# NVlabs/intrinsic3d

Measured on AMD Instinct MI355X. Metric: Gauss-Newton iterations/s at the finest SDF level, higher is better.
Workload: dtype f32

## Files before the change

intrinsic3d_amd/csrc/device/build.hip:

```cpp
#include <type_traits>
#include "kernels.hpp"
#include "reduce_device.hpp"

namespace i3d {

typedef float v4f_row __attribute__((ext_vector_type(4)));
typedef float v2f_row __attribute__((ext_vector_type(2)));
typedef float f2 __attribute__((ext_vector_type(2)));
static __device__ inline void st_row2(float2* p, float a, float b) { v2f_row v; v.x = a; v.y = b; __builtin_nontemporal_store(v, reinterpret_cast<v2f_row*>(p)); }
static __device__ inline void st_row(float4* p, float a, float b, float c, float d) { v4f_row v; v.x = a; v.y = b; v.z = c; v.w = d; __builtin_nontemporal_store(v, reinterpret_cast<v4f_row*>(p)); }

typedef float f4u __attribute__((ext_vector_type(4), aligned(4)));
typedef const __attribute__((address_space(1))) f4u* gf4u_ptr;
typedef const __attribute__((address_space(1))) float* gf_ptr;

constexpr int Q_LDS_STRIDE = 296;
struct PointShared {
    double P[3];
    double B;
    float n[3];
    float inv_len;
    float s;
    float Ls;
    float dLs[3];
// ... 449 lines not shown
                    const f2 e0 = c * (au * dxk0 + av * (y0 * r2 + c2 * dxk0)), e1 = c * (au * dxk1 + av * (y0 * r4 + c2 * dxk1)), e2 = c * (au * dxk2 + av * (y0 * r6 + c2 * dxk2));
                    const f2 e3 = c * (au * dxk3 + av * (c2 * dxk3 + (r2 + 2.0f * y0 * y0))), e4 = c * (au * dxk4 + av * (2.0f * xd * y0 + c2 * dxk4));
                    J[P_DIST + 0] -= e0.x + e0.y; J[P_DIST + 1] -= e1.x + e1.y; J[P_DIST + 2] -= e2.x + e2.y; J[P_DIST + 3] -= e3.x + e3.y; J[P_DIST + 4] -= e4.x + e4.y;
                }
                J[P_POSE + 0] = -(Wx * jr[0] + Wy * jr[3] + Wz * jr[6]);
                J[P_POSE + 1] = -(Wx * jr[1] + Wy * jr[4] + Wz * jr[7]);
                J[P_POSE + 2] = -(Wx * jr[2] + Wy * jr[5] + Wz * jr[8]);
                float finz = 0.0f;
#pragma unroll
                for (int i = 0; i < P_TOTAL; ++i) finz = __builtin_fmaf(J[i], 0.0f, finz);
                if (!(finz == 0.0f)) continue;
#pragma unroll
                for (int gq = 0; gq < 7; ++gq)
                    st_row(&r.rows[row_index(a, nout, gq, r.slots)], J[4 * gq], J[4 * gq + 1], J[4 * gq + 2], J[4 * gq + 3]);
                const size_t ro = row_scalar_index(a, nout, r.slots);
                st_row2(&r.row_jt()[row_jt_index(a, nout, r.slots)], J[28], __int_as_float(f | (vox_free ? ROW_FREE_BIT : 0)));
                st_row2(&r.row_wr[ro], roww, (float)res);
                ++nout;
            }
            }
        }
        if (WITH_J) {
            r.nrows[a] = (uint8_t)nout;
        }
        }
    }
#ifdef I3D_COST_MULTI_PROBE
    if (!WITH_J && probe_extra) cost = 0.0;
#endif
    if (!WITH_J) block_partial_d(cost, cost_out, 1, 0);
}

void launch_build(hipStream_t st, GridView g, RowView r, OptParams p, const FrameConst* frames, bool with_jacobian, double* cost_out, double* scratch,
                  const double* cam9, const LmState* lm) {
    if (r.nC <= 0) { if (!with_jacobian && cost_out) (void)hipMemsetAsync(cost_out, 0, sizeof(double), st); return; }
#ifdef I3D_COST_MULTI_PROBE
    const int blocks = with_jacobian ? (r.nC + 255) / 256 : (((r.nC + 255) / 256 + 7) / 8) * 8 * I3D_COST_MULTI_PROBE;
#else
    const int blocks = (r.nC + 255) / 256;
#endif
    double* const cost_dst = cost_out; cost_out = scratch;
    const size_t lds = (size_t)p.K * sizeof(FrameHot), qlds = (size_t)256 * Q_LDS_STRIDE;
    if (with_jacobian) {
#ifdef I3D_BUILD_VALUE_PROBE
        if (BUILD_PROBE_WAVES > 2) {
            if (!set_dynamic_lds((const void*)k_build<true, true, 2>, "k_build<true> value probe", lds, p.K)) return;
            k_build<true, true, 2><<<blocks, 256, lds, st>>>(g, r, p, frames, cost_out, nullptr, nullptr);
            return;
        }
#endif
        if (!set_dynamic_lds((const void*)k_build<true, false, 2>, "k_build<true>", qlds, p.K)) return;
        k_build<true, false, 2><<<blocks, 256, qlds, st>>>(g, r, p, frames, cost_out, nullptr, nullptr);
    } else {
        if (lds <= 48 * 1024) k_build<false, true, 2><<<blocks, 256, lds, st>>>(g, r, p, frames, cost_out, cam9, lm);
        else k_build<false, false, 2><<<blocks, 256, 0, st>>>(g, r, p, frames, cost_out, cam9, lm);
    }
    if (!with_jacobian) launch_reduce_partials(st, scratch, blocks, 1, cost_dst, nullptr, true);
}

template <bool COST>
__global__ void __launch_bounds__(256) k_weight_sums(RowView r, GridView g, double* partials) {
    double s0 = 0, s1 = 0, s2 = 0, s3 = 0, n0 = 0, n3 = 0, na = 0, c0 = 0, c1 = 0, c2 = 0, c3 = 0;
    const int N = g.N;
    for (int a = r.own0 + blockIdx.x * blockDim.x + threadIdx.x; a < r.own1 && a < r.A; a += gridDim.x * blockDim.x) {
        if (!(r.aflags[a] & F_ACTIVE)) continue;
        na += 1.0;
        const int nr = r.nrows[a];
        for (int k = 0; k < nr; ++k) {
            const float2 wr = r.row_wr[row_scalar_index(a, k, r.slots)]; const float w = wr.x;
            s0 += (double)w; if (w != 0.0f) n0 += 1.0;
            if (COST && (__float_as_int(r.row_jt()[row_jt_index(a, k, r.slots)].y) & ROW_FREE_BIT)) c0 += (double)w * ((double)wr.y * (double)wr.y);
        }
        const uint8_t rf = r.regflags[a];
        if (rf & 1) s1 += 1.0;
        if (rf & 2) s2 += 1.0;
        const int s = COST ? r.alist[a] : 0;
        const uint8_t eafree = COST ? r.ea_free[a] : 0;
        const bool er = COST && (rf & 1) && (rf & 8), es = COST && (rf & 2) && (rf & 16);
        int ring[6];
        if (er || eafree) {
#pragma unroll
            for (int d = 0; d < 6; ++d) ring[d] = g.nbr[(size_t)d * N + s];
        }
        if (er || es) {
            const double xs = g.x_sdf[s];
            if (er) {
                const double dxx = g.x_sdf[ring[0]] + g.x_sdf[ring[1]] - 2.0 * xs, dyy = g.x_sdf[ring[2]] + g.x_sdf[ring[3]] - 2.0 * xs, dzz = g.x_sdf[ring[4]] + g.x_sdf[ring[5]] - 2.0 * xs;
                const double lap = dxx + dyy + dzz; c1 += lap * lap;
            }
            if (es) { double e = xs - g.sdf0[s]; if (e == 0.0) e = 0.0000001; c2 += e * e; }
// ... 24 lines not shown
```

intrinsic3d_amd/csrc/device/gradcol.hip:

```cpp
#include "kernels.hpp"
#include "reduce_device.hpp"
#include "wave_ops.hpp"

namespace i3d {

constexpr int GC_THREADS = 384, GC_NW = GC_THREADS / 64, GC_TC = 16, GC_NPV = 27, GC_NCAM = 34;
constexpr int GC_D_CAMW = 4, GC_D_TAG = GC_D_CAMW + ((GC_NW * (GC_NCAM + 0) + 3) & ~3), GC_D_VAL = GC_D_TAG + GC_NW * GC_TC, GC_D0 = GC_D_VAL + GC_NW * GC_TC * GC_NPV;

__device__ constexpr int8_t GC_TRI_I[21] = {0, 0, 0, 0, 0, 0, 1, 1, 1, 1, 1, 2, 2, 2, 2, 3, 3, 3, 4, 4, 5};
__device__ constexpr int8_t GC_TRI_J[21] = {0, 1, 2, 3, 4, 5, 1, 2, 3, 4, 5, 2, 3, 4, 5, 3, 4, 5, 4, 5, 5};

#ifndef GC_OCC
#define GC_OCC 2
#endif
__global__ void __launch_bounds__(GC_THREADS, GC_OCC) k_eg_gradcol(GridView g, RowView r, OptParams p, GradColBuffers b, int tiles_per_block) {
    extern __shared__ float lds[];
    const int K = p.K; const size_t Acap = r.Acap;
    const int rs = (GC_NPV * K) | 1;
    const int nacc = GC_D0 + rs + GC_NCAM;
    for (int i = threadIdx.x; i < nacc; i += GC_THREADS) lds[i] = (i >= GC_D_TAG && i < GC_D_VAL) ? __int_as_float(-1) : 0.0f;
    __syncthreads();
    const int wave = __builtin_amdgcn_readfirstlane((int)(threadIdx.x >> 6));
    const int o_tag = GC_D_TAG + wave * GC_TC, o_val = GC_D_VAL + wave * (GC_TC * GC_NPV);
    int tcount = 0;
// ... 121 lines not shown
#pragma unroll
    for (int i = 0; i < GC_NCAM; ++i) {
        float v = i < 9 ? cam9[i] : camb[i - 9];
        for (int o = 32; o > 0; o >>= 1) v += __shfl_down(v, o, 64);
        if ((threadIdx.x & 63) == 0) lds[GC_D_CAMW + wave * GC_NCAM + i] = v;
    }
    __syncthreads();
    if (threadIdx.x < GC_NCAM) { float v = 0.0f; for (int w = 0; w < GC_NW; ++w) v += lds[GC_D_CAMW + w * GC_NCAM + threadIdx.x]; cam_acc[threadIdx.x] = v; }
    __syncthreads();
    float* const rowg = b.part + (size_t)blockIdx.x * b.part_stride;
    float* const rowc = rowg + b.col_off;
    for (int i = threadIdx.x; i < 6 * K; i += GC_THREADS) { const int f = i / 6; rowg[i] = lds[GC_D0 + GC_NPV * f + (i - 6 * f)]; }
    for (int i = threadIdx.x; i < 21 * K; i += GC_THREADS) { const int f = i / 21; rowc[i] = lds[GC_D0 + GC_NPV * f + 6 + (i - 21 * f)]; }
    if (threadIdx.x < 9) rowg[6 * K + threadIdx.x] = cam_acc[threadIdx.x];
    if (threadIdx.x < 34) {
        const int i = threadIdx.x;
        constexpr int8_t DIAG[9] = {0, 4, 7, 9, 10, 15, 19, 22, 24};
        rowc[21 * K + i] = i < 9 ? cam_acc[9 + DIAG[i]] : cam_acc[i];
    }
}

int launch_eg_gradcol(hipStream_t st, GridView g, RowView r, OptParams p, GradColBuffers b) {
    if (r.nC <= 0) return 0;
    static int num_cu = 0;
    if (!num_cu) { int dev = 0; (void)hipGetDevice(&dev); hipDeviceProp_t pr; (void)hipGetDeviceProperties(&pr, dev); num_cu = pr.multiProcessorCount > 0 ? pr.multiProcessorCount : 256; }
    const int ntiles = (r.nC + GC_THREADS - 1) / GC_THREADS;
    const int want = 2 * num_cu;
    const int blocks = ntiles < want ? ntiles : want;
    const int tiles_per_block = (ntiles + blocks - 1) / blocks;
    const size_t n = (size_t)(GC_D0 + ((GC_NPV * p.K) | 1) + GC_NCAM) * sizeof(float);
    if (!set_dynamic_lds((const void*)k_eg_gradcol, "k_eg_gradcol", n, p.K)) return 0;
    const int used = (ntiles + tiles_per_block - 1) / tiles_per_block;
    k_eg_gradcol<<<used, GC_THREADS, n, st>>>(g, r, p, b, tiles_per_block);
    launch_reduce_partials(st, b.cost_partials, used, 1, b.cost_out, nullptr);
    return used;
}

}
```

intrinsic3d_amd/csrc/device/kernels.hpp:

```cpp
#pragma once
#include "common.hpp"
#include "p2p_device.hpp"

namespace i3d {

struct HashTable { unsigned long long* keys; int* vals; unsigned int mask; };
void launch_sort_keys(hipStream_t st, int N, const int* keys_xyz , unsigned long long* sort_keys, int* iota);
void launch_permute_grid(hipStream_t st, int N, const int* perm, const int* keys_xyz, const double* sdf, const double* sdf_ref,
                         const double* alb, const float* w, const uint8_t* rgb,
                         int* cx, int* cy, int* cz, int* rank, double* sdf0, double* x_sdf, double* x_alb, float* f_sdf, float* f_alb,
                         float* weight, uchar4* color);
void launch_hash_build(hipStream_t st, int N, const int* cx, const int* cy, const int* cz, HashTable t);
void launch_nbr_build(hipStream_t st, int N, const int* cx, const int* cy, const int* cz, HashTable t, int* nbr);
void launch_classify(hipStream_t st, GridView g, OptParams p, int* active_flag);
void launch_compact(hipStream_t st, int N, const int* active_flag, const int* active_scan, const uint8_t* flags, int* aidx, int* alist, uint8_t* aflags);
void launch_partition_blocks(hipStream_t st, GridView g, int A, int* alist, uint8_t* aflags, int* aidx);
void launch_group_rows(hipStream_t st, int A, const uint8_t* nrows, int* gmax);
void launch_anbr(hipStream_t st, int N, int A, int Acap, const int* alist, const int* nbr, const int* aidx, int* anbr);
void launch_scatter_sh(hipStream_t st, int N, const int* rank, const double* sh_visit , float* sh );
void launch_gather_visit(hipStream_t st, int N, const int* rank, const double* x_sdf, const double* x_alb, double* out_sdf, double* out_alb);
void launch_update_fields(hipStream_t st, int N, const int* rank, const double* sdf_ref, const double* alb, const uint8_t* rgb,
                          double* x_sdf, double* x_alb, float* f_sdf, float* f_alb, uchar4* color);

void launch_observe(hipStream_t st, GridView g, RowView r, OptParams p, const FrameConst* frames, const unsigned* cull_mask = nullptr, bool prefilter = false);
constexpr int CULL_BLOCK = 8, CULL_MAX_LEVELS = 12;
struct CullPyramid { int levels, cells; int bw[CULL_MAX_LEVELS], bh[CULL_MAX_LEVELS], off[CULL_MAX_LEVELS]; };
CullPyramid cull_pyramid(int w, int h);
void launch_depth_blocks(hipStream_t st, const FrameConst* frames, int K, int w, int h, float2* out);
void launch_group_cull(hipStream_t st, GridView g, RowView r, OptParams p, const FrameConst* frames, const float2* dblocks, float4* bounds, unsigned* mask);

void launch_build(hipStream_t st, GridView g, RowView r, OptParams p, const FrameConst* frames, bool with_jacobian, double* cost_out , double* scratch,
                  const double* cam9 = nullptr, const LmState* lm = nullptr);
void launch_weight_sums(hipStream_t st, RowView r, GridView g, bool with_cost, double* sums13 , double* scratch);

enum PassMode { PASS_GRAD = 0, PASS_JTJP = 1, PASS_COLNORM = 2 };
struct Seg2 { size_t off0, off1; int n; };
struct PassBuffers {
    float* C;
    float* treg;
    double* shared;
    double* blocks;
    float* part; int part_stride;
};
struct GradColBuffers {
    float* Cg; float* Cc;
    float* tregg; float* tregc;
    float* part; int part_stride;
    int col_off;
    double* cost_partials; double* cost_out;
};
int  launch_eg_gradcol(hipStream_t st, GridView g, RowView r, OptParams p, GradColBuffers b);
int  launch_eg_pass(hipStream_t st, PassMode mode, GridView g, RowView r, OptParams p, const float* u , PassBuffers b, const PcgState* state);
void launch_sum_rows(hipStream_t st, PassMode mode, int K, const float* part, int nrows, int stride, double* shared, double* blocks);
void launch_gather(hipStream_t st, PassMode mode, RowView r, PassBuffers b, float* out );
int  launch_gather_tail(hipStream_t st, RowView r, PassBuffers b, float* out, const float* S, const float* D2, const float* v, double* dot_partials ,
                        bool dot_atomic, const PcgState* state);
void launch_reduce_partials(hipStream_t st, const double* partials, int nblk, int ncomp, double* dst, const PcgState* state, bool assign = false);
void launch_shared_finalize(hipStream_t st, size_t tail_off, int K, OptParams p, const double* shared, float* out , bool tail, const float* S, const float* D2,
                            const float* v, double* dot_out, const PcgState* state);

void launch_fill(hipStream_t st, int n, float* x, float v);
void launch_fill_d(hipStream_t st, int n, double* x, double v);
void launch_int_to_double(hipStream_t st, const int* src, double* dst);
void launch_mul(hipStream_t st, int n, const float* a, const float* b, float* out);
void launch_scale_from_colnorm(hipStream_t st, int n, const float* c, const float* freemask, float* S, float* cm);
void launch_dot(hipStream_t st, int n, const float* a, const float* b, double* out , double* scratch);
void launch_count_above2(hipStream_t st, Seg2 sg, const float* a, const float* m, float tol, double* out, double* scratch);
void launch_count_above(hipStream_t st, int n, const float* a, const float* m, float tol, double* out, double* scratch);
void launch_dot2(hipStream_t st, Seg2 sg, const float* a, const float* b, double* out , double* scratch);
void launch_mul2(hipStream_t st, Seg2 sg, const float* a, const float* b, float* out);
void launch_freemask(hipStream_t st, RowView r, OptParams p, float* mask );

void launch_pcg_init(hipStream_t st, PcgState* state, int fixed_iterations, int max_iterations, const LmState* lm = nullptr);
int  launch_pcg_step(hipStream_t st, int mode, Seg2 sg, const float* p, const float* q, float* x, float* r, const float* b, const float* D2, const float* Minv,
                     float* z, const float* S_for_inline_q, double* partials , PcgState* state);
void launch_pcg_tail_x(hipStream_t st, size_t tail_off, int K, const float* p, float* x, const PcgState* state);
void launch_pcg_tail_a(hipStream_t st, int mode, size_t tail_off, int K, const float* Minv_blocks, const float* p, const float* q, float* x, float* r, const float* b,
                       const float* D2, float* z, const double* partials, int nblk, PcgState* state,
                       double* shared_zero, int nzero, int* host_flags, int seq,
                       const P2PDev& pd);
int  launch_pcg_direction(hipStream_t st, Seg2 sg, size_t tail_off, int ntail, const float* z, float* p, const float* S, float* u, const float* D2,
                          double* d2_partials , const PcgState* state);
void launch_pcg_tail_b(hipStream_t st, size_t tail_off, int K, OptParams p, double* shared, const double* pq_slice, const double* pq_partials, int nblk,
                       const double* pq_partials2, int nblk2, bool rowwise,
                       float* q, const float* S, const float* D2, const float* v, PcgState* state, const P2PDev& pd);
struct TilePlan {
    unsigned* lnbr;
    float* eaw_sym;
    int* halo_idx; int* halo_cnt;
    int* iota; int* ext_e; int* ext_pos;
    float* qh;
    int* ext_off;
    int* overflow;
    int T, hmax;
    int tile_first, ntiles_own;
    const int* ghost_tiles; int n_ghost;
    int det;
    const unsigned short* hp_off;
    const unsigned short* hp_src;
    int pull;
};
inline int tile_plan_pull_cap(int hmax) { return 4 * hmax; }
inline int tile_plan_hmax_of(int T) { return T == 1024 ? 2048 : 1536; }
inline int tile_plan_tiles_of(int A, int T) { return (A + T - 1) / T; }
size_t tile_plan_temp_bytes(size_t nslots);
hipError_t launch_tile_plan(hipStream_t st, RowView r, TilePlan t, int hmax_limit , void* temp, size_t temp_bytes);
void launch_eaw_sym(hipStream_t st, RowView r, TilePlan t, const int* cflag );
int  launch_eg_tile(hipStream_t st, RowView r, OptParams p, const float* u, TilePlan t, double* shared, float* qacc, double* pq_partials ,
                    const PcgState* state, float* cam_partials = nullptr, int cam_stride = 0);
void launch_ext_offsets(hipStream_t st, int n, const int* ext_e, int A, int* ext_off);
void eg_tile_launch_shape(const TilePlan& t, int K, int& blocks, int& tiles_per_block);

struct LadVec;
int  eg_tile_mr_max_systems(int K);
int  launch_eg_tile_mr(hipStream_t st, RowView r, OptParams p, TilePlan t, int nsys, const int* sys, const float* u0, float* qacc0, float* qh0, double* pq0 , float* cam0, int cam_stride,
                       const PcgState* st0 , const LadVec& lv);
int  launch_eg_tile_mr_pair(hipStream_t st, RowView r, OptParams p, TilePlan t, int na, int nb, const int* sys, const float* u0, float* qacc0, float* qh0, double* pq0 , float* cam0,
                            int cam_stride, const PcgState* st0, const LadVec& lv);

struct ShardArgs {
    P2PDev pd; RimLists rim; int seq;
    int n_slice_partials;
    int n_rim_wg;
    const float* zb; float* pb; float* ub; const float* cmb; int chunk;
};
struct LadVec {
    size_t vec;
    size_t qh;
    size_t cam;
    size_t part;
    size_t mblk;
    size_t tail;
    int sysid[LADDER_MAX];
};
struct Step3Args {
    int nq; int chunk4;
    const float4* p; const float4* qacc; float4* x; float4* r; const float4* b; float4* z;
    const float4* cm; const LmState* lm;
    const int* ext_off; const int* ext_pos; const float2* qh; int e0;
    const double* pq_partials; int n_pq; const double* d2_partials; int n_d2;
    int n_slice_wg;
    int K; int fix_poses, fix_intr, fix_dist;
    const float* cam_partials; int n_cam; int cam_stride; const float* Mblk;
    const float* tp; float* tx; float* tr; const float* tb; const float* tD2; float* tz; const float* tS;
    double* step_partials;
    PcgState* cur;
    int sharded; ShardArgs sh;
    int lad_sys;
    const double* redop; int redop_stride;
};
void launch_pcg_init3(hipStream_t st, PcgState* st2 , int fixed_iterations, int max_iterations, const LmState* lm = nullptr);
int  launch_pcg_dir3(hipStream_t st, bool init, Seg2 sg, size_t tail_off, int ntail, const float* z, float* p, const float* S, float* u, const float* D2, const float* cm, const LmState* lm,
                     const double* step_partials, int n_step, double* d2_partials, const PcgState* prev, PcgState* next, int* host_flags, int seq,
                     const ShardArgs* sa = nullptr);
void launch_rim_u(hipStream_t st, const ShardArgs& sa, const PcgState* state);
int  pcg_step3_slice_wgs(int n_entries, int cap = 0);
int  pcg_step3_tail_wgs(int K);
int  launch_pcg_step3(hipStream_t st, int mode , Step3Args a);
void launch_halo_fold(hipStream_t st, RowView r, TilePlan t, float* qacc, const PcgState* state);
void launch_pcg_init_lad(hipStream_t st, PcgState* st2_all , int B, int fixed_iterations, int max_iterations, const LmState* lm);
int  launch_pcg_dir3_lad(hipStream_t st, bool init, int nsys, Seg2 sg, size_t tail_off, int ntail, const float* z0, float* p0, const float* S, float* u0, const float* tD2_0, const float* cm, const LmState* lm,
                         const double* step_partials0, int n_step, double* d2_partials0, PcgState* st2_0, int prev_parity, int* host_flags0, int seq, const LadVec& lv,
                         int n_slice_partials = 0, const double* red4_0 = nullptr );
int  launch_pcg_step3_lad(hipStream_t st, int mode, int nsys, Step3Args a, const LadVec& lv);
void launch_lad_reduce_step(hipStream_t st, int nsys, const double* step_partials0, int n_slice, double* red4_0, const LadVec& lv);
void launch_lad_reduce_op(hipStream_t st, int nsys, const float* cam_partials0, int n_cam, int cam_stride, int NS, const double* pq_partials0, int n_pq, const double* d2_partials0, int n_d2,
                          double* redop0, int redop_stride, const LadVec& lv);

void launch_need_mask(hipStream_t st, RowView r, int slice, unsigned long long* need );
void launch_halo_items(hipStream_t st, int A, int slice, int me, const unsigned long long* need, unsigned long long* items, int* count , int cap);
void launch_tile_flags(hipStream_t st, int A, int T, const int* cflag, int* tileflag );
size_t halo_sort_temp_bytes(int cap);
hipError_t launch_halo_sort(hipStream_t st, void* temp, size_t temp_bytes, const unsigned long long* in, unsigned long long* out, int n);

void launch_candidate(hipStream_t st, GridView g, RowView r, int K, float sign, const float* step, const float* S, const double* x_shared, double* xc_sdf, double* xc_alb,
                      double* xc_shared, double* norms2 , const float* mask, double* scratch, const LmState* lm = nullptr);
void launch_accept(hipStream_t st, GridView g, RowView r, const double* xc_sdf, const double* xc_alb, const LmState* lm = nullptr);
void launch_set_double(hipStream_t st, double* dst, double v);
void launch_lm_init(hipStream_t st, LmState* lm, const double* cost, const double* ngrad, const double* nfree, double radius0, LmRecord* rec, int seq);
void launch_lm_begin(hipStream_t st, LmState* lm, int K, int fix_poses, int fix_intr, int fix_dist, const double* cdiag, const double* tri, float* Mblk,
                     const float* tc, const float* tS, float* tD2, float* tMinv, LmRecord* rec, int seq);
void launch_lm_diag_dev(hipStream_t st, int n, const float* c, const float* S, const LmState* lm, float* D2, float* Minv);
void launch_cand_frames(hipStream_t st, int K, const double* xc, const FrameConst* base, FrameConst* out, const LmState* lm);
void launch_lm_decide(hipStream_t st, LmState* lm, const PcgState* ps, const double* norms2, const double* cand_cost, int attempt, int lm_steps, LmRecord* rec, int seq,
                      int lad_next = -1 , int debug_invalid = 0);
void launch_lm_begin_lad(hipStream_t st, LmState* lm, int B, int K, int fix_poses, int fix_intr, int fix_dist, const double* cdiag, const double* tri, float* Mblk, size_t mblk_stride,
                         const float* tc, const float* tS, float* tD2, size_t tail_stride, LmRecord* rec, int seq);
void launch_mark_compute(hipStream_t st, RowView r, int* flag);
void launch_compact_list(hipStream_t st, int A, const int* flag, const int* scan, int* list);

}
```

intrinsic3d_amd/csrc/device/lm_kernels.hip:

```cpp
#include "kernels.hpp"
#include "frame_math.hpp"

namespace i3d {

static __device__ inline void lm_publish(LmRecord* rec, int seq) {
    if (rec) __hip_atomic_store(&rec->seq, seq, __ATOMIC_RELEASE, __HIP_MEMORY_SCOPE_SYSTEM);
}

__global__ void k_lm_init(LmState* lm, const double* __restrict__ cost, const double* __restrict__ ngrad, const double* __restrict__ nfree, double radius0, LmRecord* rec, int seq) {
    LmState s;
    s.cost = *cost; s.radius = radius0; s.decrease_factor = 2.0; s.ngrad = *ngrad; s.nfree = *nfree;
    s.inv_radius = (float)(1.0 / radius0); s.pad0 = 0;
    s.done = 0; s.termination = 0; s.accepted = 0; s.invalid = 0; s.attempts = 0; s.successful = 0;
    if (s.nfree == 0.0 || s.ngrad == 0.0) { s.done = 1; s.termination = 1; }
    *lm = s;
    if (rec) {
        rec->final_ = s.done; rec->accepted = 0; rec->pcg_it = 0; rec->termination = s.termination; rec->kind = 0;
        rec->cost = s.cost; rec->cand_cost = 0.0; rec->model_change = 0.0; rec->rel = 0.0; rec->radius_after = s.radius; rec->ngrad = s.ngrad; rec->nfree = s.nfree;
        lm_publish(rec, seq);
    }
}
__global__ void k_set_double(double* dst, double v) { *dst = v; }
void launch_set_double(hipStream_t st, double* dst, double v) { k_set_double<<<1, 1, 0, st>>>(dst, v); }
void launch_lm_init(hipStream_t st, LmState* lm, const double* cost, const double* ngrad, const double* nfree, double radius0, LmRecord* rec, int seq) {
    k_lm_init<<<1, 1, 0, st>>>(lm, cost, ngrad, nfree, radius0, rec, seq);
}

static __device__ inline bool spd_invert_dev(int n, const double* m, double* inv) {
    double L[36];
    for (int i = 0; i < n; ++i) for (int j = 0; j <= i; ++j) {
        double s = m[i * n + j];
        for (int k = 0; k < j; ++k) s -= L[i * n + k] * L[j * n + k];
        if (i == j) { if (!(s > 0.0)) return false; L[i * n + i] = sqrt(s); } else L[i * n + j] = s / L[j * n + j];
    }
// ... 69 lines not shown
    const int NS = 6 * K + 9;
    for (int i = gid; i < NS; i += gridDim.x * blockDim.x) { float d2, mi; lm_diag(tc[i], tS[i], inv_radius, d2, mi); tD2[(size_t)j * tail_stride + i] = d2; }
}
void launch_lm_begin_lad(hipStream_t st, LmState* lm, int B, int K, int fix_poses, int fix_intr, int fix_dist, const double* cdiag, const double* tri, float* Mblk, size_t mblk_stride,
                         const float* tc, const float* tS, float* tD2, size_t tail_stride, LmRecord* rec, int seq) {
    k_lm_begin_lad<<<dim3((K + 2 + 63) / 64, B), 64, 0, st>>>(lm, B, K, fix_poses, fix_intr, fix_dist, cdiag, tri, Mblk, mblk_stride, tc, tS, tD2, tail_stride, rec, seq);
}

__global__ void k_lm_diag_dev(int n, const float* __restrict__ c, const float* __restrict__ S, const LmState* __restrict__ lm, float* __restrict__ D2, float* __restrict__ Minv) {
    if (lm->done) return;
    const float ir = lm->inv_radius;
    for (int i = blockIdx.x * blockDim.x + threadIdx.x; i < n; i += gridDim.x * blockDim.x) { float d2, mi; lm_diag(c[i], S[i], ir, d2, mi); D2[i] = d2; Minv[i] = mi; }
}
void launch_lm_diag_dev(hipStream_t st, int n, const float* c, const float* S, const LmState* lm, float* D2, float* Minv) {
    if (n <= 0) return;
    int b = (n + 255) / 256; b = b > 2048 ? 2048 : b;
    k_lm_diag_dev<<<b, 256, 0, st>>>(n, c, S, lm, D2, Minv);
}

__global__ void __launch_bounds__(64) k_cand_frames(int K, const double* __restrict__ xc, const FrameConst* __restrict__ base, FrameConst* __restrict__ out, const LmState* __restrict__ lm) {
    if (lm->done) return;
    const int f = blockIdx.x * blockDim.x + threadIdx.x;
    if (f >= K) return;
    FrameConst fc = base[f];
    double p[6];
    for (int i = 0; i < 6; ++i) p[i] = xc[6 * f + i];
    fm::frame_from_pose(p, fc);
    out[f] = fc;
}
void launch_cand_frames(hipStream_t st, int K, const double* xc, const FrameConst* base, FrameConst* out, const LmState* lm) {
    if (K > 0) k_cand_frames<<<(K + 63) / 64, 64, 0, st>>>(K, xc, base, out, lm);
}

__global__ void k_lm_decide(LmState* lm, const PcgState* __restrict__ ps, const double* __restrict__ norms2, const double* __restrict__ cand_cost_p, int attempt , int lm_steps,
                            LmRecord* rec, int seq, int lad_next, int debug_invalid) {
    if (lm->done) return;
    const int pcg_it = ps->done == 2 ? ps->it + 1 : ps->it;
    const double xbr = ps->xbr, d2xx = ps->d2xx;
    const double model_change = 0.5 * xbr + 0.5 * d2xx;
    const bool finite = !(isnan(xbr) || isinf(xbr) || isnan(d2xx) || isinf(d2xx));
    double radius = lm->radius, decrease = lm->decrease_factor, cost = lm->cost;
    const double cand = *cand_cost_p;
    int final_ = 0, accepted = 0, termination = lm->termination, invalid = lm->invalid, successful = lm->successful;
    double rel = 0.0;
    if (!finite || !(model_change > 0.0) || debug_invalid) {
        if (++invalid >= 5) { termination = 3; final_ = 1; }
        else radius *= 0.5;
    } else {
        invalid = 0;
        const double step_norm = sqrt(norms2[0]), x_norm = sqrt(norms2[1]);
        const double cost_change = cost - cand;
        if (step_norm <= 1e-8 * (x_norm + 1e-8)) { termination = 1; final_ = 1; }
        else if (fabs(cost_change) <= 1e-6 * cost) { termination = 1; final_ = 1; }
        else {
            rel = cost_change / model_change;
            if (rel > 1e-3) {
                accepted = 1; cost = cand;
                radius = fmin(1e16, radius / fmax(1.0 / 3.0, 1.0 - pow(2.0 * rel - 1.0, 3.0)));
                decrease = 2.0;
                successful += 1; termination = 2; final_ = 1;
            } else { radius = radius / decrease; decrease *= 2.0; }
        }
    }
    if (!final_ && attempt + 1 >= lm_steps) final_ = 1;
    lm->radius = radius; lm->decrease_factor = decrease; lm->cost = cost; lm->invalid = invalid; lm->successful = successful; lm->termination = termination;
    lm->attempts = lm->attempts + 1; lm->accepted = accepted; lm->done = final_;
    if (rec) {
        rec->final_ = final_; rec->accepted = accepted; rec->pcg_it = pcg_it; rec->termination = termination; rec->kind = 1;
        rec->cost = cost; rec->cand_cost = cand; rec->model_change = model_change; rec->rel = rel; rec->radius_after = radius; rec->ngrad = lm->ngrad; rec->nfree = lm->nfree;
        lm_publish(rec, seq);
    }
    if (!final_ && lad_next >= 0 && lad_next < lm->lad_n) {
        LmRecord* const nrec = rec ? rec + 1 : nullptr;
        if (radius != lm->lad_radius[lad_next]) {
            lm->done = 2;
            if (nrec) { nrec->final_ = 0; nrec->accepted = 0; nrec->pcg_it = 0; nrec->termination = termination; nrec->kind = 3; nrec->cost = cost; nrec->cand_cost = 0.0; nrec->model_change = 0.0;
                        nrec->rel = 0.0; nrec->radius_after = radius; nrec->ngrad = lm->ngrad; nrec->nfree = lm->nfree; lm_publish(nrec, seq + 1); }
        } else if (radius < 1e-32) {
            lm->termination = 1; lm->done = 1;
            if (nrec) { nrec->final_ = 1; nrec->accepted = 0; nrec->pcg_it = 0; nrec->termination = 1; nrec->kind = 2; nrec->cost = cost; nrec->cand_cost = 0.0; nrec->model_change = 0.0;
                        nrec->rel = 0.0; nrec->radius_after = radius; nrec->ngrad = lm->ngrad; nrec->nfree = lm->nfree; lm_publish(nrec, seq + 1); }
        }
    }
}
void launch_lm_decide(hipStream_t st, LmState* lm, const PcgState* ps, const double* norms2, const double* cand_cost, int attempt, int lm_steps, LmRecord* rec, int seq, int lad_next, int debug_invalid) {
    k_lm_decide<<<1, 1, 0, st>>>(lm, ps, norms2, cand_cost, attempt, lm_steps, rec, seq, lad_next, debug_invalid);
}

}
```

intrinsic3d_amd/csrc/device/operator.hip:

```cpp
#include "kernels.hpp"
#include "reduce_device.hpp"
#include "wave_ops.hpp"

namespace i3d {

#define GRID_STRIDE(n) const int stride = gridDim.x * blockDim.x; for (int i = blockIdx.x * blockDim.x + threadIdx.x; i < (n); i += stride)
static inline int vblocks(int n) { int b = (n + 255) / 256; return b < 1 ? 1 : (b > 2048 ? 2048 : b); }

__global__ void __launch_bounds__(1024) k_reduce_partials(const double* __restrict__ partials, int nblk, int ncomp, double* dst, const PcgState* __restrict__ state, int assign) {
    if (state && state->done) return;
    for (int k = 0; k < ncomp; ++k) {
        double s = 0.0;
        for (int i0 = threadIdx.x; i0 < nblk; i0 += 8 * 1024) {
            double v[8];
#pragma unroll
            for (int q = 0; q < 8; ++q) v[q] = partials[(size_t)min(i0 + q * 1024, nblk - 1) * ncomp + k];
#pragma unroll
            for (int q = 0; q < 8; ++q) if (i0 + q * 1024 < nblk) s += v[q];
        }
        const double t = block_sum_d(s);
        if (threadIdx.x == 0) dst[k] = assign ? t : dst[k] + t;
    }
}
void launch_reduce_partials(hipStream_t st, const double* partials, int nblk, int ncomp, double* dst, const PcgState* state, bool assign) {
    if (nblk > 0) k_reduce_partials<<<1, 1024, 0, st>>>(partials, nblk, ncomp, dst, state, assign ? 1 : 0);
}

constexpr int EG_THREADS = 1024;

template <int MODE>
__global__ void __launch_bounds__(EG_THREADS) k_eg_pass(GridView g, RowView r, OptParams p, PassBuffers b, int tiles_per_block, const PcgState* __restrict__ state) {
    static_assert(MODE == PASS_GRAD || MODE == PASS_COLNORM, "the operator pass has its own kernel");
    if (state && state->done) return;
    extern __shared__ float lds[];
    const int K = p.K; const size_t Acap = r.Acap;
    constexpr int NPVT = (MODE == PASS_COLNORM) ? 21 : 6, TCT = (MODE == PASS_COLNORM) ? 16 : 32, NWT = EG_THREADS / 64;
    const int rs = ((MODE == PASS_COLNORM) ? 21 * K : 6 * K) | 1;
    constexpr int NCAM = (MODE == PASS_COLNORM) ? 34 : 9;
    constexpr int D_CAMW = 4, D_TAG = D_CAMW + ((NWT * NCAM + 3) & ~3), D_VAL = D_TAG + NWT * TCT, D0 = D_VAL + NWT * TCT * NPVT;
    const int nacc = D0 + rs + NCAM;
    for (int i = threadIdx.x; i < nacc; i += EG_THREADS) lds[i] = (i >= D_TAG && i < D_VAL) ? __int_as_float(-1) : 0.0f;
    __syncthreads();
    const int wave = __builtin_amdgcn_readfirstlane((int)(threadIdx.x >> 6));
    const int o_tag = D_TAG + wave * TCT, o_val = D_VAL + wave * (TCT * NPVT);
    int tcount = 0;
    float* const cam_acc = lds + D0 + rs;
    float cam9[9];
#pragma unroll
    for (int i = 0; i < 9; ++i) cam9[i] = 0.0f;
    float camb[NCAM];
#pragma unroll
    for (int i = 0; i < NCAM; ++i) camb[i] = 0.0f;
    const float tw0 = (float)p.type_w[0];
// ... 426 lines not shown
    k_shared_finalize<<<(6 * K + 9 + 255) / 256, 256, 0, st>>>(tail_off, K, p, shared, out, tail ? 1 : 0, S, D2, v, dot_out, state);
}

__global__ void k_fill(int n, float* x, float v) { GRID_STRIDE(n) x[i] = v; }
__global__ void k_fill_d(int n, double* x, double v) { GRID_STRIDE(n) x[i] = v; }
__global__ void k_mul(int n, const float* a, const float* b, float* o) { GRID_STRIDE(n) o[i] = a[i] * b[i]; }
__global__ void k_mul2(int n, size_t seg, const float* a, const float* b, float* o) { GRID_STRIDE(2 * n) { const size_t j = i < n ? (size_t)i : (size_t)(i - n) + seg; o[j] = a[j] * b[j]; } }
__global__ void k_scale(int n, const float* c, const float* m, float* S, float* cm) { GRID_STRIDE(n) { const float v = m[i] != 0.0f ? c[i] : -1.0f; cm[i] = v; S[i] = lm_scale(v); } }
__global__ void __launch_bounds__(256) k_dot(int n, const float* a, const float* b, double* out) {
    double s = 0.0; GRID_STRIDE(n) s += (double)a[i] * (double)b[i];
    block_partial_d(s, out, 1, 0);
}
__global__ void __launch_bounds__(256) k_dot2(int n, size_t seg, const float* a, const float* b, double* out) {
    double s = 0.0; GRID_STRIDE(2 * n) { const size_t j = i < n ? (size_t)i : (size_t)(i - n) + seg; s += (double)a[j] * (double)b[j]; }
    block_partial_d(s, out, 1, 0);
}
__global__ void __launch_bounds__(256) k_count_above(int n, const float* a, const float* m, float tol, double* out) {
    double s = 0.0; GRID_STRIDE(n) s += (fabsf(a[i] * m[i]) > tol) ? 1.0 : 0.0;
    block_partial_d(s, out, 1, 0);
}
__global__ void __launch_bounds__(256) k_count_above2(int n, size_t seg, const float* a, const float* m, float tol, double* out) {
    double s = 0.0; GRID_STRIDE(2 * n) { const size_t j = i < n ? (size_t)i : (size_t)(i - n) + seg; s += (fabsf(a[j] * m[j]) > tol) ? 1.0 : 0.0; }
    block_partial_d(s, out, 1, 0);
}
void launch_fill(hipStream_t st, int n, float* x, float v) { if (n > 0) k_fill<<<vblocks(n), 256, 0, st>>>(n, x, v); }
void launch_fill_d(hipStream_t st, int n, double* x, double v) { if (n > 0) k_fill_d<<<vblocks(n), 256, 0, st>>>(n, x, v); }
__global__ void k_int_to_double(const int* src, double* dst) { *dst = (double)*src; }
void launch_int_to_double(hipStream_t st, const int* src, double* dst) { k_int_to_double<<<1, 1, 0, st>>>(src, dst); }
void launch_mul(hipStream_t st, int n, const float* a, const float* b, float* o) { if (n > 0) k_mul<<<vblocks(n), 256, 0, st>>>(n, a, b, o); }
void launch_mul2(hipStream_t st, Seg2 sg, const float* a, const float* b, float* o) {
    if (sg.n > 0) k_mul2<<<vblocks(2 * sg.n), 256, 0, st>>>(sg.n, sg.off1 - sg.off0, a + sg.off0, b + sg.off0, o + sg.off0);
}
void launch_scale_from_colnorm(hipStream_t st, int n, const float* c, const float* m, float* S, float* cm) { if (n > 0) k_scale<<<vblocks(n), 256, 0, st>>>(n, c, m, S, cm); }
void launch_dot2(hipStream_t st, Seg2 sg, const float* a, const float* b, double* out, double* scratch) {
    if (sg.n <= 0) return;
    const int blocks = vblocks(2 * sg.n) > 1024 ? 1024 : vblocks(2 * sg.n);
    k_dot2<<<blocks, 256, 0, st>>>(sg.n, sg.off1 - sg.off0, a + sg.off0, b + sg.off0, scratch);
    launch_reduce_partials(st, scratch, blocks, 1, out, nullptr);
}
void launch_count_above2(hipStream_t st, Seg2 sg, const float* a, const float* m, float tol, double* out, double* scratch) {
    if (sg.n <= 0) return;
    const int blocks = vblocks(2 * sg.n) > 1024 ? 1024 : vblocks(2 * sg.n);
    k_count_above2<<<blocks, 256, 0, st>>>(sg.n, sg.off1 - sg.off0, a + sg.off0, m + sg.off0, tol, scratch);
    launch_reduce_partials(st, scratch, blocks, 1, out, nullptr);
}
void launch_count_above(hipStream_t st, int n, const float* a, const float* m, float tol, double* out, double* scratch) {
    if (n <= 0) return;
    const int blocks = vblocks(n) > 1024 ? 1024 : vblocks(n);
    k_count_above<<<blocks, 256, 0, st>>>(n, a, m, tol, scratch);
    launch_reduce_partials(st, scratch, blocks, 1, out, nullptr);
}
void launch_dot(hipStream_t st, int n, const float* a, const float* b, double* out, double* scratch) {
    if (n <= 0) return;
    const int blocks = vblocks(n) > 1024 ? 1024 : vblocks(n);
    k_dot<<<blocks, 256, 0, st>>>(n, a, b, scratch);
    launch_reduce_partials(st, scratch, blocks, 1, out, nullptr);
}

__global__ void k_freemask(RowView r, OptParams p, float* __restrict__ mask) {
    const int A = r.A, chunk = r.chunk, nv = 2 * chunk, NP = nv + 6 * p.K + 9;
    GRID_STRIDE(NP) {
        float m;
        if (i < nv) {
            const int a = i < chunk ? i : i - chunk;
            m = (a < A && (r.aflags[a] & (i < chunk ? F_FREE_SDF : F_FREE_ALB))) ? 1.0f : 0.0f;
        }
        else if (i < nv + 6 * p.K) m = p.fix_poses ? 0.0f : 1.0f;
        else if (i < nv + 6 * p.K + 4) m = p.fix_intr ? 0.0f : 1.0f;
        else m = p.fix_dist ? 0.0f : 1.0f;
        mask[i] = m;
    }
}
void launch_freemask(hipStream_t st, RowView r, OptParams p, float* mask) { k_freemask<<<vblocks(2 * r.chunk + 6 * p.K + 9), 256, 0, st>>>(r, p, mask); }

enum { STEP_INIT = 0, STEP_NORMAL = 1, STEP_XONLY = 2, STEP_RESET = 3 };

template <int MODE, bool QINLINE>
// ... 234 lines not shown
    const size_t o = sg.off0;
    k_pcg_direction<<<blocks, 256, 0, st>>>(n4, seg4, tail_off - o, ntail, z + o, p + o, S + o, u + o, D2 + o, d2_partials, state);
    return d2_partials ? blocks : 0;
}
void launch_pcg_tail_b(hipStream_t st, size_t tail_off, int K, OptParams p, double* shared, const double* pq_slice, const double* pq_partials, int nblk,
                       const double* pq_partials2, int nblk2, bool rowwise, float* q, const float* S, const float* D2, const float* v, PcgState* state, const P2PDev& pd) {
    k_pcg_tail_b<<<1, 1024, 0, st>>>(tail_off, K, p, shared, pq_slice, pq_partials, nblk, pq_partials2, nblk2, rowwise ? 1 : 0, q, S, D2, v, state, pd);
}

__global__ void __launch_bounds__(256) k_candidate(GridView g, RowView r, int K, float sign, const float* __restrict__ step, const float* __restrict__ S,
                                                   const double* __restrict__ xsh, double* xc_sdf, double* xc_alb, double* xc_sh,
                                                   double* norms2, const float* __restrict__ mask, const LmState* __restrict__ lm) {
    if (lm && lm->done) return;
    const int A = r.A, NS = 6 * K + 9, chunk = r.chunk;
    const size_t tail = 2 * (size_t)chunk;
    double d2 = 0.0, x2 = 0.0;
    GRID_STRIDE(A + NS) {
        if (i < A) {
            const int s = r.alist[i]; const int js = vec_sdf(i, chunk), ja = js + chunk;
            const double ds = (double)sign * (double)step[js] * (double)S[js], da = (double)sign * (double)step[ja] * (double)S[ja];
            const double xs = g.x_sdf[s], xa = g.x_alb[s];
            xc_sdf[s] = xs + ds; xc_alb[s] = xa + da;
            if (mask[js] != 0.0f) { d2 += ds * ds; x2 += xs * xs; }
            if (mask[ja] != 0.0f) { d2 += da * da; x2 += xa * xa; }
        } else {
            const int t = i - A; const size_t j = tail + t;
            const double delta = (double)sign * (double)step[j] * (double)S[j];
            const double x = xsh[t]; xc_sh[t] = x + delta;
            if (mask[j] != 0.0f) { d2 += delta * delta; x2 += x * x; }
        }
    }
    block_partial_d(d2, norms2, 2, 0); block_partial_d(x2, norms2, 2, 1);
}
void launch_candidate(hipStream_t st, GridView g, RowView r, int K, float sign, const float* step, const float* S, const double* xsh, double* xc_sdf, double* xc_alb,
                      double* xc_sh, double* norms2, const float* mask, double* scratch, const LmState* lm) {
    int b = vblocks(r.A + 6 * K + 9); if (b > 1024) b = 1024;
    k_candidate<<<b, 256, 0, st>>>(g, r, K, sign, step, S, xsh, xc_sdf, xc_alb, xc_sh, scratch, mask, lm);
    launch_reduce_partials(st, scratch, b, 2, norms2, nullptr, true);
}
__global__ void k_accept(GridView g, RowView r, const double* __restrict__ xc_sdf, const double* __restrict__ xc_alb, const LmState* __restrict__ lm) {
    if (lm && !lm->accepted) return;
    GRID_STRIDE(r.A) { const int s = r.alist[i]; const double a = xc_sdf[s], b = xc_alb[s]; g.x_sdf[s] = a; g.x_alb[s] = b; g.f_sdf[s] = (float)a; g.f_alb[s] = (float)b; }
}
void launch_accept(hipStream_t st, GridView g, RowView r, const double* xc_sdf, const double* xc_alb, const LmState* lm) { if (r.A > 0) k_accept<<<vblocks(r.A), 256, 0, st>>>(g, r, xc_sdf, xc_alb, lm); }

__global__ void k_halo_pack(int n, const int* __restrict__ idx, const float* __restrict__ vec, int chunk, float* __restrict__ buf) {
    const int i = blockIdx.x * blockDim.x + threadIdx.x;
    if (i < n) { const int e = idx[i]; buf[2 * (size_t)i] = vec[e]; buf[2 * (size_t)i + 1] = vec[(size_t)chunk + e]; }
}
__global__ void k_halo_unpack(int n, const int* __restrict__ idx, const float* __restrict__ buf, int chunk, float* __restrict__ vec) {
    const int i = blockIdx.x * blockDim.x + threadIdx.x;
    if (i < n) { const int e = idx[i]; vec[e] = buf[2 * (size_t)i]; vec[(size_t)chunk + e] = buf[2 * (size_t)i + 1]; }
}
__global__ void k_halo_pack_multi(int n, const int* __restrict__ idx, const float* __restrict__ vec0, size_t stride, HaloSys sys, int nsys, int chunk, float* __restrict__ buf) {
    const int i = blockIdx.x * blockDim.x + threadIdx.x;
    if (i >= n * nsys) return;
    const int j = i / nsys, s = i - j * nsys, e = idx[j];
    const float* v = vec0 + (size_t)sys.id[s] * stride;
    buf[2 * (size_t)i] = v[e]; buf[2 * (size_t)i + 1] = v[(size_t)chunk + e];
}
__global__ void k_halo_unpack_multi(int n, const int* __restrict__ idx, const float* __restrict__ buf, size_t stride, HaloSys sys, int nsys, int chunk, float* __restrict__ vec0) {
    const int i = blockIdx.x * blockDim.x + threadIdx.x;
    if (i >= n * nsys) return;
    const int j = i / nsys, s = i - j * nsys, e = idx[j];
    float* v = vec0 + (size_t)sys.id[s] * stride;
    v[e] = buf[2 * (size_t)i]; v[(size_t)chunk + e] = buf[2 * (size_t)i + 1];
}
void launch_halo_pack_multi(hipStream_t st, int n, const int* idx, const float* vec0, size_t stride, HaloSys sys, int nsys, int chunk, float* buf) {
    if (n > 0 && nsys > 0) k_halo_pack_multi<<<(n * nsys + 255) / 256, 256, 0, st>>>(n, idx, vec0, stride, sys, nsys, chunk, buf);
}
void launch_halo_unpack_multi(hipStream_t st, int n, const int* idx, const float* buf, size_t stride, HaloSys sys, int nsys, int chunk, float* vec0) {
    if (n > 0 && nsys > 0) k_halo_unpack_multi<<<(n * nsys + 255) / 256, 256, 0, st>>>(n, idx, buf, stride, sys, nsys, chunk, vec0);
}
void launch_halo_pack(hipStream_t st, int n, const int* idx, const float* vec, int chunk, float* buf) { if (n > 0) k_halo_pack<<<(n + 255) / 256, 256, 0, st>>>(n, idx, vec, chunk, buf); }
void launch_halo_unpack(hipStream_t st, int n, const int* idx, const float* buf, int chunk, float* vec) { if (n > 0) k_halo_unpack<<<(n + 255) / 256, 256, 0, st>>>(n, idx, buf, chunk, vec); }

__global__ void k_mark_compute(RowView r, int* __restrict__ flag) {
// ... 13 lines not shown
```

intrinsic3d_amd/csrc/device/pcg_fused.hip:

```cpp
#include "kernels.hpp"
#include "reduce_device.hpp"
#include <cstring>

namespace i3d {

constexpr int PF_THREADS = 512;
constexpr int PF_MAX_WG = 512;
constexpr int PF_POSES_PER_WG = 10;

template <int NC>
static __device__ inline void reduce_partials_all(const double* __restrict__ P, int nblk, double (&tot)[NC], double* sm ,
                                                  const double* __restrict__ P2 = nullptr, int nblk2 = 0 ) {
    double v[NC];
#pragma unroll
    for (int k = 0; k < NC; ++k) v[k] = 0.0;
    for (int i = threadIdx.x; i < nblk; i += PF_THREADS) {
#pragma unroll
        for (int k = 0; k < NC; ++k) v[k] += P[(size_t)i * NC + k];
    }
    for (int i = threadIdx.x; i < nblk2; i += PF_THREADS) {
#pragma unroll
        for (int k = 0; k < NC; ++k) v[k] += P2[(size_t)i * NC + k];
    }
#pragma unroll
// ... 182 lines not shown

__global__ void __launch_bounds__(PF_THREADS) k_rim_u(ShardArgs sa, const PcgState* __restrict__ state) {
    if (state->done) return;
    const RimLists& rl = sa.rim; const unsigned e32 = p2p_pass_epoch(sa.seq, P2P_X_RESET_RIM);
    for (int j = blockIdx.x * PF_THREADS + threadIdx.x; j < rl.n_send; j += gridDim.x * PF_THREADS) {
        const int e = rl.send_idx[j], k = rl.send_peer[j];
        p2p_put_rim(sa.pd, 0, e32, k, j - rl.send_off[k], sa.ub[e], sa.ub[(size_t)sa.chunk + e]);
    }
    for (int j = blockIdx.x * PF_THREADS + threadIdx.x; j < rl.n_recv; j += gridDim.x * PF_THREADS) {
        const int e = rl.recv_idx[j], k = rl.recv_peer[j];
        float us, ua; p2p_get_rim(sa.pd, 0, e32, k, j - rl.recv_off[k], us, ua);
        sa.ub[e] = us; sa.ub[(size_t)sa.chunk + e] = ua;
    }
}
void launch_rim_u(hipStream_t st, const ShardArgs& sa, const PcgState* state) { if (sa.rim.n_send > 0 || sa.rim.n_recv > 0) k_rim_u<<<sa.n_rim_wg > 0 ? sa.n_rim_wg : 1, PF_THREADS, 0, st>>>(sa, state); }

enum { S3_INIT = 0, S3_NORMAL = 1, S3_XONLY = 2, S3_RESET = 3 };


struct S3Off { size_t v4, vo, qh2, part, cam, mblk, tail; int st, sys; };
struct S3In { float4 as, aa; int4 o; int o4; float4 x[2], p[2], b[2], cm[2], r[2]; };
template <int MODE> static __device__ inline void s3_load(const Step3Args& a, const S3Off& o, int q, S3In& v) {
    const float4* const qacc = a.qacc + o.v4; const float4* const x = a.x + o.v4; const float4* const p = a.p + o.v4; const float4* const r = a.r + o.v4;
    if (MODE == S3_NORMAL || MODE == S3_RESET) {
        v.as = qacc[q]; v.aa = qacc[q + a.chunk4];
        const int e = a.e0 + 4 * q;
        v.o = *reinterpret_cast<const int4*>(a.ext_off + e);
        v.o4 = a.ext_off[e + 4];
    }
#pragma unroll
    for (int seg = 0; seg < 2; ++seg) {
        const int i = q + seg * a.chunk4;
        v.cm[seg] = a.cm[i];
        if (MODE == S3_INIT) v.r[seg] = r[i];
        else {
            v.x[seg] = x[i];
            if (MODE != S3_RESET) v.p[seg] = p[i];
            if (MODE != S3_XONLY) { v.b[seg] = a.b[i]; if (MODE == S3_NORMAL) v.r[seg] = r[i]; }
        }
    }
}

template <int MODE, int SH>
static __device__ __forceinline__ void pcg_step3_body(const Step3Args& a, const S3Off& o) {
    __shared__ double sm[4 * 8];
    __shared__ double smx[SH == 1 ? P2P_MAX_RANKS : 1];
    __shared__ double camv[64];
    __shared__ double camred[8][64];
    __shared__ float rs[64];
    PcgState* const cur = a.cur + o.st;
    float4* const X = a.x + o.v4; float4* const R = a.r + o.v4; float4* const Z = a.z + o.v4;
    const double* const pq_partials = a.pq_partials + o.part; const double* const d2_partials = a.d2_partials + o.part; double* const step_partials = a.step_partials + o.part;
    const float2* const qh = a.qh + o.qh2; const float* const cam_partials = a.cam_partials + o.cam; const float* const Mblk = a.Mblk + o.mblk;
    const float* const tp = a.tp + o.vo; float* const tx = a.tx + o.vo; float* const tr = a.tr + o.vo; float* const tz = a.tz + o.vo; const float* const tD2 = a.tD2 + o.tail;
    const bool slice_wg = (int)blockIdx.x < a.n_slice_wg;
    const int q0 = blockIdx.x * PF_THREADS + threadIdx.x, qstride = a.n_slice_wg * PF_THREADS;
    S3In in;
    __shared__ int done_s;
    if (threadIdx.x == 0) done_s = cur->done;
    __syncthreads();
    if (done_s) return;
    const float inv_radius = o.sys >= 0 ? a.lm->lad_inv_radius[o.sys] : a.lm->inv_radius;
    float alpha = 0.0f;
    if (MODE == S3_NORMAL || MODE == S3_XONLY) {
        double t1[1];
        if (SH == 2) t1[0] = a.redop[(size_t)(o.sys < 0 ? 0 : o.sys) * a.redop_stride + 6 * a.K + 9] + d2_partials[a.n_d2];
        else reduce_partials_all<1>(pq_partials, a.n_pq, t1, sm, d2_partials, a.n_d2);
        if (SH == 1) {
            const unsigned e32 = p2p_pass_epoch(a.sh.seq, P2P_X_STEP);
            if (blockIdx.x == 0 && threadIdx.x == 0) p2p_put_double_all(a.sh.pd, 1, e32, 0, t1[0]);
            p2p_sum_all<1>(a.sh.pd, 1, e32, t1, smx);
            t1[0] += d2_partials[a.n_d2];
        }
        const double pq = t1[0];
        const double al = cur->rho / pq;
        const bool bad = !(pq > 0.0) || isinf(pq) || isinf(al);
        if (blockIdx.x == 0 && threadIdx.x == 0) { cur->pq = pq; if (bad) cur->done = 2; else cur->alpha = al; }
        if (bad) return;
        alpha = (float)al;
    }
    double s0 = 0.0, s1 = 0.0, s2 = 0.0, s3 = 0.0;
    if (slice_wg) {
        for (int q = q0; q < a.nq; q += qstride) {
            s3_load<MODE>(a, o, q, in);
            float accv[2][4];
            if (MODE == S3_NORMAL || MODE == S3_RESET) {
                const float4 as = in.as, aa = in.aa;
                accv[0][0] = as.x; accv[0][1] = as.y; accv[0][2] = as.z; accv[0][3] = as.w; accv[1][0] = aa.x; accv[1][1] = aa.y; accv[1][2] = aa.z; accv[1][3] = aa.w;
                const int ob[5] = {in.o.x, in.o.y, in.o.z, in.o.w, in.o4};
                for (int j0 = ob[0]; j0 < ob[4]; j0 += 8) {
                    int pos[8]; float2 hv[8];
#pragma unroll
                    for (int u = 0; u < 8; ++u) pos[u] = (j0 + u < ob[4]) ? a.ext_pos[j0 + u] : -1;
#pragma unroll
                    for (int u = 0; u < 8; ++u) hv[u] = pos[u] >= 0 ? qh[pos[u]] : make_float2(0.0f, 0.0f);
#pragma unroll
                    for (int u = 0; u < 8; ++u) {
                        const int j = j0 + u;
                        if (j < ob[4]) {
#pragma unroll
                            for (int k = 0; k < 4; ++k) { const bool mine = j >= ob[k] && j < ob[k + 1]; accv[0][k] += mine ? hv[u].x : 0.0f; accv[1][k] += mine ? hv[u].y : 0.0f; }
                        }
                    }
                }
            }
#pragma unroll
            for (int seg = 0; seg < 2; ++seg) {
                const int i = q + seg * a.chunk4;
                float xv[4], rv[4], svv[4], dv[4], mv[4];
                { const float4 cv = in.cm[seg]; lm_from_colnorm(cv.x, inv_radius, svv[0], dv[0], mv[0]); lm_from_colnorm(cv.y, inv_radius, svv[1], dv[1], mv[1]);
                  lm_from_colnorm(cv.z, inv_radius, svv[2], dv[2], mv[2]); lm_from_colnorm(cv.w, inv_radius, svv[3], dv[3], mv[3]); }
                if (MODE == S3_INIT) { const float4 t = in.r[seg]; rv[0] = t.x; rv[1] = t.y; rv[2] = t.z; rv[3] = t.w; }
                else {
                    const float4 xo = in.x[seg];
                    xv[0] = xo.x; xv[1] = xo.y; xv[2] = xo.z; xv[3] = xo.w;
                    float pv[4] = {0.0f, 0.0f, 0.0f, 0.0f};
                    if (MODE != S3_RESET) {
                        const float4 pp = in.p[seg]; pv[0] = pp.x; pv[1] = pp.y; pv[2] = pp.z; pv[3] = pp.w;
#pragma unroll
                        for (int k = 0; k < 4; ++k) xv[k] += alpha * pv[k];
                        X[i] = make_float4(xv[0], xv[1], xv[2], xv[3]);
                    }
                    if (MODE == S3_XONLY) continue;
                    const float4 bb = in.b[seg];
                    const float bv[4] = {bb.x, bb.y, bb.z, bb.w};
                    float qq[4];
#pragma unroll
                    for (int k = 0; k < 4; ++k) qq[k] = svv[k] * accv[seg][k] + dv[k] * (MODE == S3_NORMAL ? pv[k] : xv[k]);
                    if (MODE == S3_NORMAL) { const float4 ro = in.r[seg]; rv[0] = ro.x - alpha * qq[0]; rv[1] = ro.y - alpha * qq[1]; rv[2] = ro.z - alpha * qq[2]; rv[3] = ro.w - alpha * qq[3]; }
                    else { rv[0] = bv[0] - qq[0]; rv[1] = bv[1] - qq[1]; rv[2] = bv[2] - qq[2]; rv[3] = bv[3] - qq[3]; }
                    R[i] = make_float4(rv[0], rv[1], rv[2], rv[3]);
#pragma unroll
                    for (int k = 0; k < 4; ++k) { const double xd = xv[k]; s1 += xd * ((double)bv[k] + (double)rv[k]); s2 += xd * (double)rv[k]; s3 += (double)dv[k] * xd * xd; }
                }
                const float zv[4] = {mv[0] * rv[0], mv[1] * rv[1], mv[2] * rv[2], mv[3] * rv[3]};
                Z[i] = make_float4(zv[0], zv[1], zv[2], zv[3]);
#pragma unroll
                for (int k = 0; k < 4; ++k) s0 += (double)rv[k] * (double)zv[k];
            }
        }
    } else {
        const int K = a.K, tw = (int)blockIdx.x - a.n_slice_wg, n_pose_wg = (K + PF_POSES_PER_WG - 1) / PF_POSES_PER_WG;
        int col0, ncol;
        if (tw < n_pose_wg) { col0 = 6 * PF_POSES_PER_WG * tw; const int c1 = min(6 * K, col0 + 6 * PF_POSES_PER_WG); ncol = c1 - col0; }
        else { col0 = 6 * K; ncol = 9; }
        const int t = threadIdx.x;
        if (MODE == S3_NORMAL || MODE == S3_RESET) {
            const int g = t / 64, c = t % 64;
            double v = 0.0;
            if (SH != 2 && c < ncol) for (int w = g; w < a.n_cam; w += 8) v += (double)cam_partials[(size_t)w * a.cam_stride + col0 + c];
            camred[g][c] = v;
            __syncthreads();
            if (t < ncol) {
                double s = 0.0; for (int gg = 0; gg < 8; ++gg) s += camred[gg][t];
                if (SH == 2) s = a.redop[(size_t)(o.sys < 0 ? 0 : o.sys) * a.redop_stride + col0 + t];
                if (SH == 1) {
                    const unsigned e32 = p2p_pass_epoch(a.sh.seq, MODE == S3_RESET ? P2P_X_RESET_STEP : P2P_X_STEP);
                    p2p_put_double_all(a.sh.pd, 1, e32, 1 + col0 + t, s);
                    s = 0.0; for (int j = 0; j < a.sh.pd.L.world; ++j) s += p2p_get_double(a.sh.pd, 1, e32, j, 1 + col0 + t);
                }
                camv[t] = s;
            }
            __syncthreads();
        }
        if (t < ncol) {
            const int i = col0 + t;
            const bool fixed = i < 6 * K ? a.fix_poses : (i < 6 * K + 4 ? a.fix_intr : a.fix_dist);
            float ri;
            if (MODE == S3_INIT) ri = tr[i];
            else {
                float xi = tx[i];
                if (MODE != S3_RESET) { xi += alpha * tp[i]; tx[i] = xi; }
                if (MODE == S3_XONLY) ri = 0.0f;
                else {
                    const float vv = MODE == S3_NORMAL ? tp[i] : xi;
                    const float qi = a.tS[i] * (fixed ? 0.0f : (float)camv[t]) + tD2[i] * vv;
                    ri = MODE == S3_NORMAL ? tr[i] - alpha * qi : a.tb[i] - qi;
                    tr[i] = ri;
                    const double xd = xi; s1 += xd * ((double)a.tb[i] + (double)ri); s2 += xd * (double)ri; s3 += (double)tD2[i] * xd * xd;
                }
            }
            rs[t] = ri;
        }
        if (MODE == S3_XONLY) return;
        __syncthreads();
        if (t < ncol) {
            const int i = col0 + t;
            int base, n, row; const float* M;
            if (i < 6 * K) { const int f = i / 6; base = 6 * f; n = 6; row = i - base; M = Mblk + 36 * f; }
            else if (i < 6 * K + 4) { base = 6 * K; n = 4; row = i - base; M = Mblk + 36 * K; }
            else { base = 6 * K + 4; n = 5; row = i - base; M = Mblk + 36 * K + 16; }
            float s = 0.0f;
            for (int j = 0; j < n; ++j) s += M[row * n + j] * rs[base - col0 + j];
            tz[i] = s; s0 += (double)rs[t] * (double)s;
        }
    }
    if (MODE == S3_XONLY) return;
    block_partial_d(s0, step_partials, 4, 0); block_partial_d(s1, step_partials, 4, 1); block_partial_d(s2, step_partials, 4, 2); block_partial_d(s3, step_partials, 4, 3);
}
template <int MODE, int SH>
__global__ void __launch_bounds__(PF_THREADS) k_pcg_step3(Step3Args a) { const S3Off o{0, 0, 0, 0, 0, 0, 0, 0, -1}; pcg_step3_body<MODE, SH>(a, o); }
template <int MODE, bool COLL>
// ... 96 lines not shown
```

intrinsic3d_amd/csrc/device/reduce_device.hpp:

```cpp
#pragma once
#include <hip/hip_runtime.h>

namespace i3d {

static __device__ inline double block_sum_d(double v) {
    __shared__ double sm_red[16];
    for (int o = 32; o > 0; o >>= 1) v += __shfl_down(v, o, 64);
    if ((threadIdx.x & 63) == 0) sm_red[threadIdx.x >> 6] = v;
    __syncthreads();
    double t = 0.0;
    if (threadIdx.x == 0) for (int i = 0; i < (int)((blockDim.x + 63) >> 6); ++i) t += sm_red[i];
    __syncthreads();
    return t;
}
static __device__ inline void block_partial_d(double v, double* partials, int ncomp, int comp) {
    const double t = block_sum_d(v);
    if (threadIdx.x == 0) partials[(size_t)blockIdx.x * ncomp + comp] = t;
}

}
```

intrinsic3d_amd/csrc/device/tile_pass.hip:

```cpp
#include <cstring>
#include <climits>
#include "kernels.hpp"
#include "reduce_device.hpp"
#include "wave_ops.hpp"
#include "tile_device.hpp"
#include <rocprim/rocprim.hpp>

namespace i3d {

constexpr int TP_PLAN_LIST = 2048;
constexpr int TP_NONE = 0x7f7f7f7f;
__device__ __host__ inline int tp_dir(int j) {
    constexpr int8_t D[18] = {NB_PY, NB_P2Y, NB_PYZ, NB_PZ, NB_P2Z, NB_PX, NB_PXY, NB_PXZ, NB_P2X, NB_MX, NB_MY, NB_MZ,
                              NB_M2Y, NB_MYZ, NB_M2Z, NB_MXY, NB_MXZ, NB_M2X};
    return D[j];
}

__global__ void __launch_bounds__(1024) k_tile_plan(RowView r, int T, int hmax, int hlimit , int tile_first, const int* __restrict__ tile_list, unsigned* __restrict__ lnbr,
                                                    int* __restrict__ halo_idx, int* __restrict__ halo_cnt, int* __restrict__ overflow) {
    __shared__ int hkeys[4096];
    __shared__ int hlist[TP_PLAN_LIST];
    __shared__ int cnt;
    const int tile = tile_list ? tile_list[blockIdx.x] : tile_first + (int)blockIdx.x, base = tile * T, a = base + threadIdx.x;
    const bool in = (int)threadIdx.x < T && a < r.A;
// ... 450 lines not shown
        if (cam_partials) cam_partials[(size_t)blockIdx.x * cam_stride + q] = v;
        else if (v != 0.0f) atomicAdd(&shared[q], (double)v);
    }
    if (pq_partials) block_partial_d(pq_l[i], pq_partials, 1, 0);
#undef pq_l
#undef hp_list
#undef hp_offs
#undef o_tag
#undef o_val
#undef upose
#undef u_s
#undef u_a
#undef qh_s
#undef qh_a
#undef tr_l
#undef C_l
#undef ui
#undef Cme
}

__global__ void __launch_bounds__(256) k_halo_fold(int n, const int* __restrict__ ext_e, const int* __restrict__ ext_pos, const float* __restrict__ qh,
                                                   float* __restrict__ qacc, int chunk, const PcgState* __restrict__ state) {
    if (state && state->done) return;
    const int i = blockIdx.x * blockDim.x + threadIdx.x;
    if (i >= n) return;
    const int e = ext_e[i];
    if (e >= TP_NONE || (i > 0 && ext_e[i - 1] == e)) return;
    float s = 0.0f, al = 0.0f;
    for (int j = i; j < n && ext_e[j] == e; ++j) { const float2 v = reinterpret_cast<const float2*>(qh)[ext_pos[j]]; s += v.x; al += v.y; }
    qacc[e] += s; qacc[chunk + e] += al;
}

__global__ void k_iota(int n, int* __restrict__ x) { const int i = blockIdx.x * blockDim.x + threadIdx.x; if (i < n) x[i] = i; }

size_t tile_plan_temp_bytes(size_t nslots) {
    size_t bytes = 0;
    (void)rocprim::radix_sort_pairs(nullptr, bytes, (const int*)nullptr, (int*)nullptr, (const int*)nullptr, (int*)nullptr, nslots, 0, 32, (hipStream_t)0);
    return bytes;
}

hipError_t launch_tile_plan(hipStream_t st, RowView r, TilePlan t, int hmax_limit, void* temp, size_t temp_bytes) {
    const int ntiles = tile_plan_tiles_of(r.A, t.T);
    if (ntiles <= 0) return hipSuccess;
    hipError_t e = hipMemsetAsync(t.overflow, 0, sizeof(int), st); if (e != hipSuccess) return e;
    const int n = ntiles * t.hmax;
    const int hlimit = (hmax_limit > 0 && hmax_limit < t.hmax) ? hmax_limit : t.hmax;
    const bool all = t.tile_first == 0 && t.ntiles_own >= ntiles;
    if (!all) { e = hipMemsetAsync(t.halo_idx, 0x7f, sizeof(int) * (size_t)n, st); if (e != hipSuccess) return e;
                e = hipMemsetAsync(t.halo_cnt, 0, sizeof(int) * (size_t)ntiles, st); if (e != hipSuccess) return e; }
    if (t.ntiles_own > 0) k_tile_plan<<<t.ntiles_own, 1024, 0, st>>>(r, t.T, t.hmax, hlimit, t.tile_first, nullptr, t.lnbr, t.halo_idx, t.halo_cnt, t.overflow);
    if (t.n_ghost > 0) k_tile_plan<<<t.n_ghost, 1024, 0, st>>>(r, t.T, t.hmax, hlimit, 0, t.ghost_tiles, t.lnbr, t.halo_idx, t.halo_cnt, t.overflow);
    if (t.hp_off) {
        unsigned short* off = const_cast<unsigned short*>(t.hp_off); unsigned short* src = const_cast<unsigned short*>(t.hp_src);
        if (t.T == 1024) { if (t.ntiles_own > 0) k_tile_pull_plan<1024, 2048><<<t.ntiles_own, 1024, 0, st>>>(r, t.tile_first, nullptr, t.lnbr, t.halo_cnt, off, src, t.overflow);
                           if (t.n_ghost > 0) k_tile_pull_plan<1024, 2048><<<t.n_ghost, 1024, 0, st>>>(r, 0, t.ghost_tiles, t.lnbr, t.halo_cnt, off, src, t.overflow); }
        else { if (t.ntiles_own > 0) k_tile_pull_plan<512, 1536><<<t.ntiles_own, 512, 0, st>>>(r, t.tile_first, nullptr, t.lnbr, t.halo_cnt, off, src, t.overflow);
               if (t.n_ghost > 0) k_tile_pull_plan<512, 1536><<<t.n_ghost, 512, 0, st>>>(r, 0, t.ghost_tiles, t.lnbr, t.halo_cnt, off, src, t.overflow); }
    }
    k_iota<<<(n + 255) / 256, 256, 0, st>>>(n, t.iota);
    int key_bits = 32;
    for (int b = 1; b < 32; ++b) { const unsigned mask = (1u << b) - 1u; if ((1u << b) >= (unsigned)r.A && ((unsigned)TP_NONE & mask) >= (unsigned)r.A) { key_bits = b; break; } }
    e = rocprim::radix_sort_pairs(temp, temp_bytes, (const int*)t.halo_idx, t.ext_e, (const int*)t.iota, t.ext_pos, (size_t)n, 0, key_bits, st);
    if (e != hipSuccess) return e;
    if (t.ext_off) launch_ext_offsets(st, n, t.ext_e, r.chunk, t.ext_off);
    return hipGetLastError();
}

void launch_eaw_sym(hipStream_t st, RowView r, TilePlan t, const int* cflag) { if (r.A > 0) k_eaw_sym<<<(r.A + 255) / 256, 256, 0, st>>>(r, cflag, t.eaw_sym); }

struct EgtShape { bool tables, pull; int reps, per_cu, blocks, tiles_per_block; size_t lds; };
template <int T, int HMAX>
static EgtShape egt_shape(const TilePlan& t, int K, int num_cu) {
    const int nshared = 6 * K + 9, rs = (6 * K) | 1;
    EgtShape s; s.tables = t.det != 0; s.pull = s.tables || (t.pull && t.hp_off != nullptr);
    const bool det = s.tables, pull = s.pull;
    constexpr int NW = T / 64, TC = T == 1024 ? 64 : 32;
    const int det_words = det ? 4 + ((NW * 9 + 3) & ~3) + NW * TC * 7 : 0;
    auto lds_bytes = [&](int reps) { const int nacc = det_words + reps * rs + 9; const int o_upose = (nacc + 3) & ~3, o_u = (o_upose + nshared + 3) & ~3;
                                     return (size_t)(o_u + 2 * (T + HMAX + 1) + 2 * HMAX + T + 4 + 12 * T + 2 * T  + (pull ? (HMAX + 4) / 2 : 0) ) * sizeof(float); };
    const size_t budget = (T == 512 ? 79 : 158) * 1024;
    s.reps = s.tables ? 1 : 4;
    while (s.reps > 1 && lds_bytes(s.reps) > budget) s.reps >>= 1;
    s.lds = lds_bytes(s.reps);
    s.per_cu = (T == 512 && s.lds <= budget) ? 2 : 1;
    const int ntl = t.ntiles_own + t.n_ghost;
    s.blocks = 0; s.tiles_per_block = 0;
    if (ntl > 0) {
        s.blocks = ntl < s.per_cu * num_cu ? ntl : s.per_cu * num_cu;
        s.tiles_per_block = (ntl + s.blocks - 1) / s.blocks;
        if (ntl > s.blocks && ntl < 2 * s.blocks) { s.tiles_per_block = 1; s.blocks = ntl; }
    }
    return s;
// ... 52 lines not shown
```

intrinsic3d_amd/csrc/host/context.cpp:

```cpp
#include "context.hpp"
#include "../device/frame_math.hpp"
#include <rocprim/rocprim.hpp>
#include <algorithm>

using namespace i3d;

static thread_local std::string g_create_error;

namespace i3d {

int ctx_fail(i3d_context* c, int code, const std::string& msg) { if (c) c->err = msg; else g_create_error = msg; return code; }
int ctx_hip(i3d_context* c, hipError_t e, const char* what) {
    return ctx_fail(c, I3D_ERR_HIP, std::string(what) + " -> " + hipGetErrorString(e));
}

int ctx_launch_check(i3d_context* c) {
    char msg[256];
    if (take_launch_error(msg, sizeof(msg))) return ctx_fail(c, I3D_ERR_CAPACITY, msg);
    const hipError_t e = hipGetLastError();
    return e == hipSuccess ? I3D_OK : ctx_hip(c, e, "kernel launch");
}

int ensure_pinned(i3d_context* c, size_t n) {
    if (n <= c->h_pinned_n) return I3D_OK;
// ... 88 lines not shown
    if (c->h_pinned) (void)hipHostFree(c->h_pinned);
    if (c->h_pcg) (void)hipHostFree(c->h_pcg);
    if (c->h_flags) (void)hipHostFree(c->h_flags);
    if (c->h_lmrec) (void)hipHostFree(c->h_lmrec);
    for (auto e : c->ev_asm) if (e) (void)hipEventDestroy(e);
    for (auto e : c->pcg_ev) if (e) (void)hipEventDestroy(e);
    delete c->comm;
    if (c->stream) (void)hipStreamDestroy(c->stream);
    delete c;
}

int i3d_set_grid(i3d_context* c, const i3d_grid_view* gv) {
    if (!c || !gv || gv->num_voxels <= 0 || !gv->keys || !gv->sdf || !gv->sdf_refined || !gv->albedo || !gv->weight || !gv->color)
        return ctx_fail(c, I3D_ERR_INVALID_ARGUMENT, "i3d_set_grid: null grid or empty voxel list");
    if (gv->num_voxels > (1ll << 30)) return ctx_fail(c, I3D_ERR_CAPACITY, "i3d_set_grid: more than 2^30 voxels");
    CTX_HIP(c, hipSetDevice(c->device));
    const int N = (int)gv->num_voxels;
    hipStream_t st = c->stream;
    GridStaging g;
    CTX_HIP(c, g.kxyz.alloc((size_t)3 * N)); CTX_HIP(c, g.sdf.alloc(N)); CTX_HIP(c, g.sdf_ref.alloc(N)); CTX_HIP(c, g.alb.alloc(N)); CTX_HIP(c, g.w.alloc(N)); CTX_HIP(c, g.rgb.alloc((size_t)3 * N));
    CTX_HIP(c, hipMemcpyAsync(g.kxyz.p, gv->keys, sizeof(int) * 3 * (size_t)N, hipMemcpyHostToDevice, st));
    CTX_HIP(c, hipMemcpyAsync(g.sdf.p, gv->sdf, sizeof(double) * (size_t)N, hipMemcpyHostToDevice, st));
    CTX_HIP(c, hipMemcpyAsync(g.sdf_ref.p, gv->sdf_refined, sizeof(double) * (size_t)N, hipMemcpyHostToDevice, st));
    CTX_HIP(c, hipMemcpyAsync(g.alb.p, gv->albedo, sizeof(double) * (size_t)N, hipMemcpyHostToDevice, st));
    CTX_HIP(c, hipMemcpyAsync(g.w.p, gv->weight, sizeof(float) * (size_t)N, hipMemcpyHostToDevice, st));
    CTX_HIP(c, hipMemcpyAsync(g.rgb.p, gv->color, (size_t)3 * N, hipMemcpyHostToDevice, st));
    return set_grid_device(c, N, gv->voxel_size, gv->truncation, g);
}

}

namespace i3d {
int set_grid_device(i3d_context* c, int N, float voxel_size, float truncation, GridStaging& g) {
    c->N = N; c->voxel_size = voxel_size; c->truncation = truncation; c->have_grid = false; c->have_sh = false; c->have_subvolumes = false; c->assembled = false;
    c->render_bricks_ok = false;
    c->slots = 0;
    hipStream_t st = c->stream;
    DevBuf<int> perm, iota; DevBuf<unsigned long long> skeys, skeys2;
    CTX_HIP(c, perm.alloc(N)); CTX_HIP(c, iota.alloc(N)); CTX_HIP(c, skeys.alloc(N)); CTX_HIP(c, skeys2.alloc(N));
    launch_sort_keys(st, N, g.kxyz.p, skeys.p, iota.p);
    size_t tmp_bytes = 0;
    CTX_HIP(c, rocprim::radix_sort_pairs(nullptr, tmp_bytes, skeys.p, skeys2.p, iota.p, perm.p, (size_t)N, 0, 64, st));
    DevBuf<unsigned char> tmp; CTX_HIP(c, tmp.alloc(tmp_bytes));
    CTX_HIP(c, rocprim::radix_sort_pairs(tmp.p, tmp_bytes, skeys.p, skeys2.p, iota.p, perm.p, (size_t)N, 0, 64, st));
    auto fit = [&](auto& buf, size_t n) -> hipError_t { if (buf.n != n) buf.release(); return buf.alloc(n); };
    CTX_HIP(c, fit(c->cx, N)); CTX_HIP(c, fit(c->cy, N)); CTX_HIP(c, fit(c->cz, N)); CTX_HIP(c, fit(c->rank, N));
    CTX_HIP(c, fit(c->sdf0, N)); CTX_HIP(c, fit(c->x_sdf, N)); CTX_HIP(c, fit(c->x_alb, N)); CTX_HIP(c, fit(c->xc_sdf, N)); CTX_HIP(c, fit(c->xc_alb, N));
    CTX_HIP(c, fit(c->f_sdf, N)); CTX_HIP(c, fit(c->f_alb, N)); CTX_HIP(c, fit(c->weight, N)); CTX_HIP(c, fit(c->color, N));
    CTX_HIP(c, fit(c->flags, N)); CTX_HIP(c, fit(c->aidx, N)); CTX_HIP(c, fit(c->alist, N)); CTX_HIP(c, fit(c->aflag, N)); CTX_HIP(c, fit(c->ascan, N));
    CTX_HIP(c, fit(c->sh, (size_t)9 * N)); CTX_HIP(c, fit(c->nbr, (size_t)NUM_NBR * N));
    launch_permute_grid(st, N, perm.p, g.kxyz.p, g.sdf.p, g.sdf_ref.p, g.alb.p, g.w.p, g.rgb.p, c->cx.p, c->cy.p, c->cz.p, c->rank.p, c->sdf0.p,
                        c->x_sdf.p, c->x_alb.p, c->f_sdf.p, c->f_alb.p, c->weight.p, c->color.p);
    CTX_HIP(c, hipMemcpyAsync(c->xc_sdf.p, c->x_sdf.p, sizeof(double) * (size_t)N, hipMemcpyDeviceToDevice, st));
    CTX_HIP(c, hipMemcpyAsync(c->xc_alb.p, c->x_alb.p, sizeof(double) * (size_t)N, hipMemcpyDeviceToDevice, st));
    unsigned int cap = 1; while (cap < (unsigned int)N * 2u) cap <<= 1;
    CTX_HIP(c, fit(c->hkeys, cap)); CTX_HIP(c, fit(c->hvals, cap)); c->hmask = cap - 1;
    CTX_HIP(c, hipMemsetAsync(c->hkeys.p, 0xff, sizeof(unsigned long long) * (size_t)cap, st));
    HashTable t{c->hkeys.p, c->hvals.p, cap - 1};
    launch_hash_build(st, N, c->cx.p, c->cy.p, c->cz.p, t);
    launch_nbr_build(st, N, c->cx.p, c->cy.p, c->cz.p, t, c->nbr.p);
    CTX_HIP(c, hipMemsetAsync(c->sh.p, 0, sizeof(float) * 9 * (size_t)N, st));
    size_t sb = 0;
    CTX_HIP(c, rocprim::exclusive_scan(nullptr, sb, c->aflag.p, c->ascan.p, 0, (size_t)N, rocprim::plus<int>(), st));
    c->scan_tmp.release(); CTX_HIP(c, c->scan_tmp.alloc(sb ? sb : 1)); c->scan_tmp_bytes = sb;
    CTX_HIP(c, hipStreamSynchronize(st));
    CTX_HIP(c, hipGetLastError());
    c->have_grid = true;
    return I3D_OK;
}
}

extern "C" {

int i3d_get_grid(i3d_context* c, double* sdf_refined, double* albedo) {
    if (!c || !c->have_grid) return ctx_fail(c, I3D_ERR_STATE, "i3d_get_grid: no grid");
    CTX_HIP(c, hipSetDevice(c->device));
    const int N = c->N;
    DevBuf<double> a, b; CTX_HIP(c, a.alloc(N)); CTX_HIP(c, b.alloc(N));
    launch_gather_visit(c->stream, N, c->rank.p, c->x_sdf.p, c->x_alb.p, a.p, b.p);
    if (sdf_refined) CTX_HIP(c, hipMemcpyAsync(sdf_refined, a.p, sizeof(double) * (size_t)N, hipMemcpyDeviceToHost, c->stream));
    if (albedo) CTX_HIP(c, hipMemcpyAsync(albedo, b.p, sizeof(double) * (size_t)N, hipMemcpyDeviceToHost, c->stream));
    CTX_HIP(c, hipStreamSynchronize(c->stream));
    return I3D_OK;
}

int i3d_update_grid(i3d_context* c, const double* sdf_refined, const double* albedo, const uint8_t* color) {
    if (!c || !c->have_grid) return ctx_fail(c, I3D_ERR_STATE, "i3d_update_grid: no grid");
    CTX_HIP(c, hipSetDevice(c->device));
    const int N = c->N;
    DevBuf<double> a, b; DevBuf<uint8_t> col;
    if (sdf_refined) { CTX_HIP(c, a.alloc(N)); CTX_HIP(c, hipMemcpyAsync(a.p, sdf_refined, sizeof(double) * (size_t)N, hipMemcpyHostToDevice, c->stream)); }
    if (albedo) { CTX_HIP(c, b.alloc(N)); CTX_HIP(c, hipMemcpyAsync(b.p, albedo, sizeof(double) * (size_t)N, hipMemcpyHostToDevice, c->stream)); }
    if (color) { CTX_HIP(c, col.alloc((size_t)3 * N)); CTX_HIP(c, hipMemcpyAsync(col.p, color, (size_t)3 * N, hipMemcpyHostToDevice, c->stream)); }
    launch_update_fields(c->stream, N, c->rank.p, a.p, b.p, col.p, c->x_sdf.p, c->x_alb.p, c->f_sdf.p, c->f_alb.p, c->color.p);
    CTX_HIP(c, hipStreamSynchronize(c->stream));
    c->assembled = false;
    return I3D_OK;
}

int i3d_set_frames(i3d_context* c, int32_t K, int32_t levels, const int32_t* widths, const int32_t* heights,
                   const float* const* lum, const float* const* depth, const uint8_t* const* bgr) {
    if (!c || K <= 0 || levels <= 0 || !widths || !heights || !lum || !depth) return ctx_fail(c, I3D_ERR_INVALID_ARGUMENT, "i3d_set_frames: bad arguments");
    CTX_HIP(c, hipSetDevice(c->device));
    c->have_frames = false; c->K = K; c->levels = levels; c->cull_level = -1;
    c->slots = 0; c->assembled = false;
    c->fw.assign(widths, widths + levels); c->fh.assign(heights, heights + levels);
    c->lum.clear(); c->depth.clear(); c->bgr.clear();
    c->lum.resize((size_t)K * levels); c->depth.resize((size_t)K * levels); c->bgr.resize((size_t)K * levels);
    for (int f = 0; f < K; ++f) for (int l = 0; l < levels; ++l) {
        const size_t k = (size_t)f * levels + l, px = (size_t)widths[l] * heights[l];
        if (!lum[k] || !depth[k]) return ctx_fail(c, I3D_ERR_INVALID_ARGUMENT, "i3d_set_frames: null image");
        CTX_HIP(c, c->lum[k].alloc(px + 4));        CTX_HIP(c, c->depth[k].alloc(px));
        CTX_HIP(c, hipMemcpyAsync(c->lum[k].p, lum[k], px * sizeof(float), hipMemcpyHostToDevice, c->stream));
        CTX_HIP(c, hipMemcpyAsync(c->depth[k].p, depth[k], px * sizeof(float), hipMemcpyHostToDevice, c->stream));
        if (bgr && bgr[k]) { CTX_HIP(c, c->bgr[k].alloc(px * 3)); CTX_HIP(c, hipMemcpyAsync(c->bgr[k].p, bgr[k], px * 3, hipMemcpyHostToDevice, c->stream)); }
    }
    CTX_HIP(c, c->d_frames.alloc(K)); CTX_HIP(c, c->d_frames_cand.alloc(K));
    CTX_HIP(c, hipStreamSynchronize(c->stream));
    c->have_frames = true;
    if ((int)c->poses.size() != 6 * K) { c->poses.assign((size_t)6 * K, 0.0); c->have_camera = false; }
    return I3D_OK;
}

int i3d_set_camera(i3d_context* c, const double* intr, const double* dist, const double* poses) {
    if (!c || !intr || !dist || !poses) return ctx_fail(c, I3D_ERR_INVALID_ARGUMENT, "i3d_set_camera: null pointer");
    if (!c->have_frames) return ctx_fail(c, I3D_ERR_STATE, "i3d_set_camera: set the keyframes first");
// ... 80 lines not shown
```

intrinsic3d_amd/csrc/host/context.hpp:

```cpp
#pragma once
#include <functional>
#include <string>
#include <vector>
#include <cstring>
#include <cmath>
#include "../device/kernels.hpp"
#include "../device/render_kernels.hpp"
#include "../device/track_kernels.hpp"
#include "../device/query_kernels.hpp"
#include "../device/register_kernels.hpp"
#include "../device/track_sdf_kernels.hpp"
#include "comm.hpp"
#include "../../../include/intrinsic3d_hip.h"

namespace i3d {

template <class T>
struct DevBuf {
    T* p = nullptr; size_t n = 0;
    DevBuf() = default;
    DevBuf(const DevBuf&) = delete; DevBuf& operator=(const DevBuf&) = delete;
    DevBuf(DevBuf&& o) noexcept : p(o.p), n(o.n) { o.p = nullptr; o.n = 0; }
    DevBuf& operator=(DevBuf&& o) noexcept { if (this != &o) { release(); p = o.p; n = o.n; o.p = nullptr; o.n = 0; } return *this; }
    ~DevBuf() { release(); }
// ... 104 lines not shown
    int  deterministic = -1;
    int  ladder = LADDER_MAX;
    bool ladder_mr = true, ladder_mr1 = false, ladder_pair = true; int ladder_group = 3;
    bool egt_mr1 = false;
    int  egt_tile = 0;
    int  hmax_limit = 0, hmax_limit_1024 = 0;
    bool halo_pull = false, no_tile = false, gradcol = true, cost0 = true;
    int  no_cull = 0;
    int  debug_invalid_attempt = -1;
    int  sh_slab = 0;
};

struct Timing {
    bool on = false;
    unsigned mask = ~0u;
    double ms[I3D_K_COUNT] = {0};
    long long launches[I3D_K_COUNT] = {0};
    std::vector<float> each[I3D_K_COUNT];
    struct Pending { hipEvent_t a, b; int cat; };
    std::vector<Pending> pending;
    std::vector<hipEvent_t> pool;
};

}

struct i3d_context {
    int device = 0;
    hipStream_t stream = nullptr;
    std::string err;

    int N = 0; float voxel_size = 0, truncation = 0;
    i3d::DevBuf<int> cx, cy, cz, rank, nbr, aidx, alist, aflag, ascan;
    i3d::DevBuf<double> sdf0, x_sdf, x_alb, xc_sdf, xc_alb;
    i3d::DevBuf<float> f_sdf, f_alb, weight, sh;
    i3d::DevBuf<uchar4> color;
    i3d::DevBuf<uint8_t> flags;
    i3d::DevBuf<unsigned char> scan_tmp; size_t scan_tmp_bytes = 0;
    i3d::DevBuf<unsigned long long> hkeys; i3d::DevBuf<int> hvals; unsigned int hmask = 0;
    bool have_grid = false, have_sh = false;
    i3d::DevBuf<unsigned> render_bits; i3d::DevBuf<int> render_bounds; int render_lo[3] = {0, 0, 0}, render_dim[3] = {0, 0, 0}; bool render_bricks_ok = false;
    i3d::DevBuf<float> render_planes; i3d::DevBuf<i3d::RenderStatsDev> render_stats;
    i3d::TrackBuffers track;
    i3d::DevBuf<unsigned char> query_scratch;
    i3d::DevBuf<unsigned char> register_scratch; int register_row_cap = i3d::REGISTER_MAX_ROWS;
    i3d::TrackSdfBuffers track_sdf; int track_batch_frames = 0;
    i3d::DevBuf<double> track_sdf_intensity;
    std::vector<unsigned long long> sv_keys; std::vector<double> sv_sh; float sv_size = 0.0f; bool have_subvolumes = false;

    int K = 0, levels = 0;
    std::vector<int> fw, fh;
    std::vector<i3d::DevBuf<float>> lum, depth;
    std::vector<i3d::DevBuf<uint8_t>> bgr;
    i3d::DevBuf<i3d::FrameConst> d_frames, d_frames_cand;
    bool have_frames = false;

    double intr[4] = {0, 0, 0, 0}, dist[5] = {0, 0, 0, 0, 0};
    std::vector<double> poses;
    bool have_camera = false;

    int Acap = 0, slots = 0, A = 0; long long n_active = 0;
    i3d::Comm* comm = nullptr; int chunk = 1, own0 = 0, own1 = 0, nC = 0;
    i3d::DevBuf<int> clist, cflag, cscan;
    i3d::HaloPlan halo; i3d::DevBuf<unsigned long long> need_mask, halo_items, halo_sorted; i3d::DevBuf<int> halo_count, halo_send_idx, halo_recv_idx, halo_send_peer, halo_recv_peer, halo_offs, tile_flag, ghost_tiles;
    i3d::DevBuf<float> halo_send_buf, halo_recv_buf; i3d::DevBuf<unsigned char> halo_temp; int n_ghost_tiles = 0, slice = 0;
    i3d::DevBuf<int> obs_frame, anbr; i3d::DevBuf<float> obs_w, ea_w, C, treg;
    i3d::DevBuf<float4> rows; i3d::DevBuf<float2> row_wr;
// ... 8 lines not shown
    bool ladder_lists = false;
    i3d::SolverSwitches sw;
    bool mr1_serial = false;
    int ladder_max = 1;
    int ladder_hint = 0, ladder_hint_prev = 0;
    i3d::LadVec lad{};
    i3d::DevBuf<float> lad_vec;
    i3d::DevBuf<float> lad_qh, lad_cam, lad_mblk, lad_tail;
    i3d::DevBuf<double> lad_part;
    i3d::DevBuf<double> lad_red;
    i3d::DevBuf<i3d::PcgState> lad_st;
    long long lad_batches = 0, lad_streams = 0, lad_system_passes = 0, lad_resyncs = 0, lad_wasted = 0;
    long long lad_pass_live[7] = {0, 0, 0, 0, 0, 0, 0}, lad_paired = 0;
    double t_add_end = 0.0;
    bool deterministic = false;
    int tile_T = 0;
    int plan_T() const { return tile_T > 0 ? tile_T : (sw.egt_tile == 512 ? 512 : 1024); }
    int plan_hmax_limit() const { return plan_T() == 512 ? sw.hmax_limit : sw.hmax_limit_1024; }
    i3d::TilePlan tile_plan() const {
        const int T = plan_T();
        const bool sh = comm && (comm->world > 1 || comm->force);
        const int t0 = sh ? own0 / T : 0, t1 = sh ? (own1 + T - 1) / T : i3d::tile_plan_tiles_of(A, T);
        return i3d::TilePlan{tp_lnbr.p, tp_eaw.p, tp_halo_idx.p, tp_halo_cnt.p, tp_iota.p, tp_ext_e.p, tp_ext_pos.p, tp_qh.p, tp_ext_off.p, tp_overflow.p, T, i3d::tile_plan_hmax_of(T), t0, t1 > t0 ? t1 - t0 : 0,
                             ghost_tiles.p, sh ? n_ghost_tiles : 0, deterministic ? 1 : 0, (halo_pull || ladder_lists) ? tp_hp_off.p : nullptr, (halo_pull || ladder_lists) ? tp_hp_src.p : nullptr, halo_pull ? 1 : 0};
    }

    i3d::DevBuf<float> v_mask, v_c, v_S, v_cm, v_D2, v_Minv, v_b, v_x, v_r, v_p, v_z, v_q, v_u, v_acc, v_tmp, v_qacc;
    i3d::DevBuf<float> Minv_blocks;
    i3d::DevBuf<double> d_shared, d_blocks, d_scal, d_xshared, d_xcshared;
    i3d::DevBuf<i3d::PcgState> d_pcg, d_pcg2; i3d::DevBuf<double> d_partials; i3d::PcgState* h_pcg = nullptr; hipEvent_t pcg_ev[2] = {nullptr, nullptr};
    int* h_flags = nullptr; int* d_flags = nullptr; int pcg_seq = 1024;
    i3d::DevBuf<i3d::LmState> d_lm; i3d::LmRecord* h_lmrec = nullptr; i3d::LmRecord* d_lmrec = nullptr; int lm_seq = 1;
    i3d::DevBuf<double> d_cam_c, d_cam_H;
    hipEvent_t ev_asm[2] = {nullptr, nullptr};
    long long n_syncs = 0;
    double* h_pinned = nullptr; size_t h_pinned_n = 0;

    i3d::OptParams last_params; bool assembled = false;
    long long last_sizes[6] = {0, 0, 0, 0, 0, 0};
    i3d::Timing timing;

    i3d::GridView grid_view() const;
    i3d::RowView row_view() const;
};

namespace i3d {

int ctx_fail(i3d_context* c, int code, const std::string& msg);
int ctx_hip(i3d_context* c, hipError_t e, const char* what);
int ctx_launch_check(i3d_context* c);
#define CTX_HIP(c, expr) do { hipError_t _e = (expr); if (_e != hipSuccess) return i3d::ctx_hip((c), _e, #expr); } while (0)
void build_frame_consts(const i3d_context* c, int level, const double* poses, std::vector<FrameConst>& out);
int ensure_pinned(i3d_context* c, size_t n);
bool timing_begin(i3d_context* c, int cat);
void timing_end(i3d_context* c);
void timing_flush(i3d_context* c);
struct TimedScope { i3d_context* c; bool active; TimedScope(i3d_context* c_, int cat) : c(c_), active(timing_begin(c_, cat)) {} ~TimedScope() { if (active) timing_end(c); } };

struct GridStaging { DevBuf<int> kxyz; DevBuf<double> sdf, sdf_ref, alb; DevBuf<float> w; DevBuf<uint8_t> rgb; };
int set_grid_device(i3d_context* c, int N, float voxel_size, float truncation, GridStaging& st);

int render_ensure_bricks(i3d_context* c);
RenderGrid render_grid(const i3d_context* c, bool refined);
inline RenderGrid field_grid(const i3d_context* c, bool refined) {
    return RenderGrid{HashTable{c->hkeys.p, c->hvals.p, c->hmask}, c->nbr.p, c->N, c->weight.p, refined ? c->x_sdf.p : c->sdf0.p, c->x_alb.p, c->sh.p,
                      (double)c->voxel_size, nullptr, {0, 0, 0}, {0, 0, 0}};
// ... 19 lines not shown
```

intrinsic3d_amd/csrc/host/solver.cpp:

```cpp
#include "context.hpp"
#include <rocprim/rocprim.hpp>
#include <chrono>
#include <cstdlib>
#include <limits>
#include <algorithm>

namespace i3d {

#ifdef I3D_MR_PHASES
void mr_phase_report_now();
#endif
#ifdef I3D_MR_BLOCKTIME
void mr_blocktime_report_now();
#endif

static double now_s() { return std::chrono::duration<double>(std::chrono::steady_clock::now().time_since_epoch()).count(); }

static OptParams make_params(const i3d_context* c, const i3d_optimizer_config& cfg, const double* intr, const double* dist) {
    OptParams p; std::memset(&p, 0, sizeof(p));
    p.thres_shell = cfg.thres_shell; p.lambda_a = cfg.lambda_a; p.K = c->K; p.level = cfg.rgbd_level;
    p.pyr_scale = 1.0 / std::pow(2.0, cfg.rgbd_level);
    p.occlusion = cfg.occlusion_distance;
    p.use_er = (cfg.lambda_r0 > 0.0 && cfg.lambda_r1 > 0.0); p.use_es = (cfg.lambda_s0 > 0.0 && cfg.lambda_s1 > 0.0); p.use_ea = cfg.lambda_a > 0.0;
    for (int i = 0; i < 4; ++i) { p.intr[i] = intr[i]; p.cam_f[i] = (float)(intr[i] * p.pyr_scale); }
// ... 6 lines not shown
}

static double varying_lambda(int it, int n, double l0, double l1) {
    if (n <= 1) return l0;
    return l0 + ((l1 - l0) / (double)(n - 1)) * (double)it;
}

constexpr int HALO_CAP = 1 << 20;
constexpr int AUX_PART_ROWS = 320;
static size_t aux_part_stride(int K) { return ((size_t)21 * K + 34 + 3) & ~(size_t)3; }
constexpr int GC_PART_ROWS = 1024;
static size_t gc_col_off(int K) { return ((size_t)6 * K + 9 + 3) & ~(size_t)3; }
static size_t gc_part_stride(int K) { return gc_col_off(K) + aux_part_stride(K); }
constexpr int PCG_SEQ_STRIDE = 1024;
constexpr int LM_REC_SLOTS = 64;

static hipError_t sync_stream(i3d_context* c) { ++c->n_syncs; return hipStreamSynchronize(c->stream); }

static int alloc_rows(i3d_context* c, int slots) {
    const size_t Acap = (size_t)c->N;
    c->Acap = (int)Acap; c->slots = slots;
    CTX_HIP(c, c->obs_frame.alloc(Acap * slots)); CTX_HIP(c, c->obs_w.alloc(Acap * slots));
    { const size_t nrow = ((Acap + 63) / 64) * 64 * (size_t)slots;
      CTX_HIP(c, c->rows.alloc(nrow / 64 * ROW_BLOCK_F4)); CTX_HIP(c, c->row_wr.alloc(nrow)); }
    CTX_HIP(c, c->aflags.alloc(Acap)); CTX_HIP(c, c->nrows.alloc(Acap)); CTX_HIP(c, c->gmax.alloc(Acap / 64 + 2)); CTX_HIP(c, c->anbr.alloc(Acap * NUM_NBR));
    CTX_HIP(c, c->cull_bounds.alloc(Acap / 64 + 2)); CTX_HIP(c, c->cull_mask.alloc((Acap / 64 + 2) * (size_t)((c->K + 31) / 32)));
    CTX_HIP(c, c->regflags.alloc(Acap)); CTX_HIP(c, c->ea_free.alloc(Acap)); CTX_HIP(c, c->ea_w.alloc(Acap * 6));
    CTX_HIP(c, c->C.alloc(Acap * P_VOX)); CTX_HIP(c, c->treg.alloc(Acap * 8)); CTX_HIP(c, c->aux_part.alloc((size_t)AUX_PART_ROWS * aux_part_stride(c->K)));
    CTX_HIP(c, c->C2.alloc(Acap * P_VOX)); CTX_HIP(c, c->treg2.alloc(Acap * 8)); CTX_HIP(c, c->gc_part.alloc((size_t)GC_PART_ROWS * gc_part_stride(c->K)));
    {
      const size_t nt = (size_t)tile_plan_tiles_of((int)Acap, 512);
      const size_t nh = std::max(nt * (size_t)tile_plan_hmax_of(512), (size_t)tile_plan_tiles_of((int)Acap, 1024) * (size_t)tile_plan_hmax_of(1024));
      CTX_HIP(c, c->tp_lnbr.alloc(Acap * LNBR_WORDS)); CTX_HIP(c, c->tp_eaw.alloc(Acap * 6)); CTX_HIP(c, c->tp_halo_idx.alloc(nh)); CTX_HIP(c, c->tp_halo_cnt.alloc(nt)); CTX_HIP(c, c->tp_iota.alloc(nh));
      CTX_HIP(c, c->tp_ext_e.alloc(nh)); CTX_HIP(c, c->tp_ext_pos.alloc(nh)); CTX_HIP(c, c->tp_qh.alloc(2 * nh)); CTX_HIP(c, c->tp_overflow.alloc(1));
      CTX_HIP(c, c->tp_ext_off.alloc(Acap + (size_t)SHARD_ALIGN * ((c->comm ? c->comm->world : 1) + 1) + 8));
      CTX_HIP(c, c->cam_part.alloc((size_t)2048 * (((size_t)6 * c->K + 9 + 3) & ~(size_t)3)));
      CTX_HIP(c, c->tp_temp.alloc(tile_plan_temp_bytes(nt * (size_t)tile_plan_hmax_of(1024)))); }
    const int world_a = c->comm ? c->comm->world : 1;
    const size_t NP = 2 * ((size_t)c->N + (size_t)SHARD_ALIGN * (world_a + 1)) + 6 * (size_t)c->K + 9;
    for (DevBuf<float>* v : {&c->v_mask, &c->v_c, &c->v_S, &c->v_cm, &c->v_D2, &c->v_Minv, &c->v_b, &c->v_x, &c->v_r, &c->v_p, &c->v_z, &c->v_q, &c->v_u, &c->v_acc, &c->v_tmp, &c->v_qacc})
        { const bool fresh = v->n < NP || !v->p; CTX_HIP(c, v->alloc(NP)); if (fresh) CTX_HIP(c, hipMemsetAsync(v->p, 0, sizeof(float) * v->n, c->stream)); }
    CTX_HIP(c, c->Minv_blocks.alloc((size_t)36 * c->K + 16 + 25));
    CTX_HIP(c, c->d_shared.alloc((size_t)6 * c->K + 9 + 1)); CTX_HIP(c, c->d_blocks.alloc((size_t)21 * c->K + 25));
    CTX_HIP(c, c->clist.alloc(Acap)); CTX_HIP(c, c->cflag.alloc(Acap)); CTX_HIP(c, c->cscan.alloc(Acap));
    if (c->comm) {
        const size_t cap = HALO_CAP;
        CTX_HIP(c, c->need_mask.alloc(Acap)); CTX_HIP(c, c->halo_items.alloc(cap)); CTX_HIP(c, c->halo_sorted.alloc(cap)); CTX_HIP(c, c->halo_count.alloc(1));
        CTX_HIP(c, c->halo_send_idx.alloc(cap)); CTX_HIP(c, c->halo_recv_idx.alloc(cap)); CTX_HIP(c, c->halo_send_peer.alloc(cap)); CTX_HIP(c, c->halo_recv_peer.alloc(cap)); CTX_HIP(c, c->halo_offs.alloc(2 * P2P_MAX_RANKS)); CTX_HIP(c, c->halo_send_buf.alloc((size_t)HALO_MULTI_MAX * (2 * cap))); CTX_HIP(c, c->halo_recv_buf.alloc((size_t)HALO_MULTI_MAX * (2 * cap)));
        CTX_HIP(c, c->halo_temp.alloc(halo_sort_temp_bytes((int)cap)));
        const size_t nt = (size_t)tile_plan_tiles_of((int)Acap, 512) + 1; CTX_HIP(c, c->tile_flag.alloc(nt)); CTX_HIP(c, c->ghost_tiles.alloc(nt));
    }
    CTX_HIP(c, c->d_scal.alloc(32)); CTX_HIP(c, c->d_xshared.alloc((size_t)6 * c->K + 9)); CTX_HIP(c, c->d_xcshared.alloc((size_t)6 * c->K + 9));
    CTX_HIP(c, c->d_pcg.alloc(1)); CTX_HIP(c, c->d_pcg2.alloc(2));
    CTX_HIP(c, c->d_partials.alloc((Acap / 256 + 2048) * 9));
    if (!c->h_pcg) CTX_HIP(c, hipHostMalloc((void**)&c->h_pcg, 2 * sizeof(PcgState), hipHostMallocDefault));
    for (auto& e : c->pcg_ev) if (!e) CTX_HIP(c, hipEventCreateWithFlags(&e, hipEventDisableTiming));
    if (!c->h_flags) { CTX_HIP(c, hipHostMalloc((void**)&c->h_flags, 32 * sizeof(int), hipHostMallocMapped | hipHostMallocCoherent));
                       for (int i = 0; i < 32; ++i) c->h_flags[i] = -1;
                       CTX_HIP(c, hipHostGetDevicePointer((void**)&c->d_flags, c->h_flags, 0)); }
    CTX_HIP(c, c->d_lm.alloc(1)); CTX_HIP(c, c->d_cam_c.alloc((size_t)6 * c->K + 9)); CTX_HIP(c, c->d_cam_H.alloc((size_t)21 * c->K + 25));
    if (!c->h_lmrec) { CTX_HIP(c, hipHostMalloc((void**)&c->h_lmrec, LM_REC_SLOTS * sizeof(LmRecord), hipHostMallocMapped | hipHostMallocCoherent));
                       std::memset(c->h_lmrec, 0, LM_REC_SLOTS * sizeof(LmRecord));
                       CTX_HIP(c, hipHostGetDevicePointer((void**)&c->d_lmrec, c->h_lmrec, 0)); }
    for (auto& e : c->ev_asm) if (!e) CTX_HIP(c, hipEventCreate(&e));
    return ensure_pinned(c, 64 + (size_t)27 * c->K + 64);
}

struct Layout { int A, K, NS, chunk, world, rank, slice; Seg2 own; size_t tail_off, NP; };
static Layout layout_of(const i3d_context* c) {
    Layout L; L.A = c->A; L.K = c->K; L.NS = 6 * c->K + 9; L.chunk = c->chunk; L.world = c->comm ? c->comm->world : 1; L.rank = c->comm ? c->comm->rank : 0;
    L.slice = L.chunk / L.world;
    L.own = Seg2{(size_t)L.rank * L.slice, (size_t)L.chunk + (size_t)L.rank * L.slice, L.slice};
    L.tail_off = 2 * (size_t)L.chunk; L.NP = L.tail_off + L.NS;
    return L;
}
static bool sharded(const i3d_context* c) { return c->comm && (c->comm->world > 1 || c->comm->force); }
static bool one_stream_gradcol(const i3d_context* c) { return !sharded(c) && c->sw.gradcol; }
static bool cost_from_sums(const i3d_context* c) { return c->sw.cost0 && !one_stream_gradcol(c); }

void read_switches(i3d_context* c) {
    auto env = [](const char* name) { return std::getenv(name); };
    auto is = [&](const char* name, char v) { const char* e = env(name); return e && e[0] == v; };
    auto num = [&](const char* name, int unset) { const char* e = env(name); return e ? std::atoi(e) : unset; };
    auto clamp = [](int v, int lo, int hi) { return v < lo ? lo : (v > hi ? hi : v); };
    SolverSwitches w;
    { const char* e = env("I3D_DETERMINISTIC"); w.deterministic = e ? (e[0] == '1' ? 1 : 0) : -1; }
    w.ladder = clamp(num("I3D_LADDER", LADDER_MAX), 1, LADDER_MAX);
    w.ladder_mr = !is("I3D_LADDER_MR", '0');
    w.ladder_mr1 = is("I3D_LADDER_MR1", '1');
    w.ladder_group = clamp(num("I3D_LADDER_GROUP", 3), 1, 3);
    w.ladder_pair = !is("I3D_LADDER_PAIR", '0');
    w.egt_mr1 = is("I3D_EGT_MR1", '1');
    { const char* e = env("I3D_EGT_TILE"); w.egt_tile = e ? (std::atoi(e) == 512 ? 512 : 1024) : 0; }
// ... 207 lines not shown
    if (st) { for (int t = 0; t < 4; ++t) { st->rows[t] = (int64_t)(sums[4 + t] + 0.5); st->weight_sum[t] = sums[t]; st->type_weight[t] = p.type_w[t]; } st->valid_voxels = c->n_active; }
    c->last_sizes[0] = c->n_active; for (int t = 0; t < 4; ++t) c->last_sizes[1 + t] = (long long)(sums[4 + t] + 0.5);
    c->last_params = p; c->assembled = true;
    { float ms = 0.0f; c->t_add_end = (hipEventElapsedTime(&ms, c->ev_asm[0], c->ev_asm[1]) == hipSuccess) ? (double)ms * 1e-3 : -1.0; }
    { const int lrc = ctx_launch_check(c); if (lrc) return lrc; }
    return I3D_OK;
}

static int run_pass(i3d_context* c, PassMode mode, const OptParams& p, const float* u, float* out ) {
    hipStream_t s = c->stream; GridView g = c->grid_view(); RowView r = c->row_view(); const Layout L = layout_of(c);
    const int stride = (int)aux_part_stride(c->K);
    PassBuffers b{c->C.p, c->treg.p, c->d_shared.p, c->d_blocks.p, c->aux_part.p, stride};
    CTX_HIP(c, hipMemsetAsync(c->d_shared.p, 0, sizeof(double) * ((size_t)L.NS + 1), s));
    if (mode == PASS_COLNORM) CTX_HIP(c, hipMemsetAsync(c->d_blocks.p, 0, sizeof(double) * (21 * (size_t)c->K + 25), s));
    if (mode == PASS_JTJP && c->tile_ok && !sharded(c)) {
        const int NSP = (L.NS + 3) & ~3; int rows = 0;
        { TimedScope t(c, I3D_K_EG_PASS); rows = launch_eg_tile(s, r, p, u, c->tile_plan(), nullptr, out, nullptr, nullptr, c->cam_part.p, NSP); }
        { TimedScope t(c, I3D_K_GATHER); launch_halo_fold(s, r, c->tile_plan(), out, nullptr); }
        { TimedScope t(c, I3D_K_VECTOR); launch_mul(s, 2 * c->chunk, c->v_mask.p, out, out);
          if (rows > 0) launch_sum_rows(s, PASS_JTJP, c->K, c->cam_part.p, rows, NSP, c->d_shared.p, c->d_blocks.p); }
    } else {
        int rows = 0;
        { TimedScope t(c, mode == PASS_JTJP ? I3D_K_EG_PASS : I3D_K_EG_AUX); rows = launch_eg_pass(s, mode, g, r, p, u, b, nullptr);
          if (rows > AUX_PART_ROWS) return ctx_fail(c, I3D_ERR_CAPACITY, "run_pass: more workgroups than rows of the camera partial buffer");
          if (rows > 0) launch_sum_rows(s, mode, c->K, c->aux_part.p, rows, stride, c->d_shared.p, c->d_blocks.p); }
        { TimedScope t(c, I3D_K_GATHER); launch_gather(s, mode, r, b, out); }
    }
    { int rc = allreduce(c, c->d_shared.p, (size_t)L.NS); if (rc) return rc; }
    if (mode == PASS_COLNORM) { int rc = allreduce(c, c->d_blocks.p, 21 * (size_t)c->K + 25); if (rc) return rc; }
    { TimedScope t(c, I3D_K_VECTOR); launch_shared_finalize(s, L.tail_off, c->K, p, c->d_shared.p, out, false, nullptr, nullptr, nullptr, nullptr, nullptr); }
    return I3D_OK;
}

template <class F> static int run_gradcol(i3d_context* c, const OptParams& p, F between) {
    hipStream_t s = c->stream; GridView g = c->grid_view(); RowView r = c->row_view(); const Layout L = layout_of(c);
    const int stride = (int)gc_part_stride(c->K), col_off = (int)gc_col_off(c->K);
    GradColBuffers gb{c->C.p, c->C2.p, c->treg.p, c->treg2.p, c->gc_part.p, stride, col_off, c->d_partials.p, c->d_scal.p + 16};
    CTX_HIP(c, hipMemsetAsync(c->d_scal.p + 16, 0, sizeof(double), s));
    CTX_HIP(c, hipMemsetAsync(c->d_shared.p, 0, sizeof(double) * ((size_t)L.NS + 1), s));
    CTX_HIP(c, hipMemsetAsync(c->d_blocks.p, 0, sizeof(double) * (21 * (size_t)c->K + 25), s));
    int rows = 0;
    { TimedScope t(c, I3D_K_EG_AUX); rows = launch_eg_gradcol(s, g, r, p, gb);
      if (rows > GC_PART_ROWS) return ctx_fail(c, I3D_ERR_CAPACITY, "run_gradcol: more workgroups than rows of the camera partial buffer");
      if (rows > 0) launch_sum_rows(s, PASS_COLNORM, c->K, c->gc_part.p + col_off, rows, stride, c->d_shared.p, c->d_blocks.p); }
    { PassBuffers b{c->C2.p, c->treg2.p, c->d_shared.p, c->d_blocks.p, nullptr, 0};
      TimedScope t(c, I3D_K_GATHER); launch_gather(s, PASS_COLNORM, r, b, c->v_c.p); }
    { TimedScope t(c, I3D_K_VECTOR); launch_shared_finalize(s, L.tail_off, c->K, p, c->d_shared.p, c->v_c.p, false, nullptr, nullptr, nullptr, nullptr, nullptr); }
    { int rc = between(); if (rc) return rc; }
    CTX_HIP(c, hipMemsetAsync(c->d_shared.p, 0, sizeof(double) * ((size_t)L.NS + 1), s));
    { TimedScope t(c, I3D_K_EG_AUX); if (rows > 0) launch_sum_rows(s, PASS_GRAD, c->K, c->gc_part.p, rows, stride, c->d_shared.p, c->d_blocks.p); }
    { PassBuffers b{c->C.p, c->treg.p, c->d_shared.p, c->d_blocks.p, nullptr, 0};
      TimedScope t(c, I3D_K_GATHER); launch_gather(s, PASS_GRAD, r, b, c->v_acc.p); }
    { TimedScope t(c, I3D_K_VECTOR); launch_shared_finalize(s, L.tail_off, c->K, p, c->d_shared.p, c->v_acc.p, false, nullptr, nullptr, nullptr, nullptr, nullptr); }
    return I3D_OK;
}

static int dot_dev(i3d_context* c, const float* a, const float* b, double* slot) {
    const Layout L = layout_of(c);
    CTX_HIP(c, hipMemsetAsync(slot, 0, sizeof(double), c->stream));
    { TimedScope t(c, I3D_K_VECTOR); launch_dot2(c->stream, L.own, a, b, slot, c->d_partials.p); }
    { int rc = allreduce(c, slot, 1); if (rc) return rc; }
    { TimedScope t(c, I3D_K_VECTOR); launch_dot(c->stream, L.NS, a + L.tail_off, b + L.tail_off, slot, c->d_partials.p); }
    return I3D_OK;
}

static int count_above_dev(i3d_context* c, const float* a, const float* m, float tol, double* slot) {
    const Layout L = layout_of(c);
    CTX_HIP(c, hipMemsetAsync(slot, 0, sizeof(double), c->stream));
    { TimedScope t(c, I3D_K_VECTOR); launch_count_above2(c->stream, L.own, a, m, tol, slot, c->d_partials.p); }
    { int rc = allreduce(c, slot, 1); if (rc) return rc; }
    { TimedScope t(c, I3D_K_VECTOR); launch_count_above(c->stream, L.NS, a + L.tail_off, m + L.tail_off, tol, slot, c->d_partials.p); }
    return I3D_OK;
}

static int eval_cost_launch(i3d_context* c, const OptParams& p, bool candidate, const FrameConst* frames, const double* cam9 = nullptr, const LmState* lm = nullptr) {
    GridView g = c->grid_view();
    if (candidate) { g.x_sdf = c->xc_sdf.p; g.x_alb = c->xc_alb.p; }
    { TimedScope t(c, I3D_K_COST); launch_build(c->stream, g, c->row_view(), p, frames, false, c->d_scal.p + 16, c->d_partials.p, cam9, lm); }
    return allreduce(c, c->d_scal.p + 16, 1);
}
static int eval_cost(i3d_context* c, const OptParams& p, bool candidate, const FrameConst* frames, double* cost) {
    int rc = eval_cost_launch(c, p, candidate, frames); if (rc) return rc;
    rc = read_doubles(c, c->d_scal.p + 16, 1, cost); if (rc) return rc;
    if (sharded(c) && c->comm->health(c->stream)) return ctx_fail(c, I3D_ERR_COMM, "cost evaluation: a peer-to-peer exchange timed out (a rank stopped taking part)");
    return I3D_OK;
}

static int wait_pass(i3d_context* c, const int* ring, int want, const char* stalled, bool* done) {
    const double t_wait = now_s();
    while (__atomic_load_n(&ring[0], __ATOMIC_ACQUIRE) != want) {
        if (now_s() - t_wait > 30.0) { CTX_HIP(c, sync_stream(c)); if (__atomic_load_n(&ring[0], __ATOMIC_ACQUIRE) != want) return ctx_fail(c, I3D_ERR_HIP, stalled); }
    }
    *done = __atomic_load_n(&ring[1], __ATOMIC_ACQUIRE) != 0;
    return I3D_OK;
}

static int pcg_solve(i3d_context* c, const i3d_optimizer_config& cfg, const OptParams& p, const PcgState** final_state) {
    hipStream_t s = c->stream;
    const Layout L = layout_of(c);
    const int K = c->K; const bool multi = sharded(c), tiled = c->tile_ok;
    GridView g = c->grid_view(); RowView r = c->row_view();
    PassBuffers pb{c->C.p, c->treg.p, c->d_shared.p, c->d_blocks.p, c->aux_part.p, (int)aux_part_stride(c->K)};
    PcgState* st = c->d_pcg.p;
    double* pq_slot = c->d_shared.p + L.NS;
    const size_t to = L.tail_off; const Seg2 own = L.own;
    { TimedScope t(c, I3D_K_VECTOR); launch_fill(s, (int)L.NP, c->v_x.p, 0.0f); launch_pcg_init(s, st, cfg.pcg_fixed_iterations, 500, c->d_lm.p); }
    CTX_HIP(c, hipMemcpyAsync(c->v_r.p, c->v_b.p, sizeof(float) * L.NP, hipMemcpyDeviceToDevice, s));
    double* const step_part = c->d_partials.p; double* const pq_part = c->d_partials.p + 4 * 2048; double* const d2_part = pq_part + 1024;
    int n_pq = 0, n_step = 0, n_d2 = 0;
    P2PDev pd; std::memset(&pd, 0, sizeof(pd));
    const bool fused = multi && tiled && c->comm->device_reduce(&pd) && L.NS + 1 <= pd.L.red_cap;
    if (!fused) pd.on = 0;
// ... 70 lines not shown
    Step3Args a; std::memset(&a, 0, sizeof(a));
    auto c4 = [&](const float* v) { return reinterpret_cast<const float4*>(v + own.off0); };
    auto m4 = [&](float* v) { return reinterpret_cast<float4*>(v + own.off0); };
    a.nq = own.n >> 2; a.chunk4 = (int)((own.off1 - own.off0) >> 2);
    a.p = c4(pv); a.qacc = c4(q); a.x = m4(x); a.r = m4(r); a.b = c4(c->v_b.p); a.z = m4(z); a.cm = c4(c->v_cm.p); a.lm = c->d_lm.p;
    a.ext_off = tp.ext_off; a.ext_pos = tp.ext_pos; a.qh = reinterpret_cast<const float2*>(qh); a.e0 = (int)own.off0;
    a.pq_partials = pq; a.d2_partials = d2; a.n_pq = 0; a.n_d2 = 0;
    a.n_slice_wg = pcg_step3_slice_wgs(own.n, wg_cap);
    a.K = c->K; a.fix_poses = p.fix_poses; a.fix_intr = p.fix_intr; a.fix_dist = p.fix_dist;
    a.cam_partials = cam; a.n_cam = 0; a.cam_stride = (L.NS + 3) & ~3; a.Mblk = Mblk;
    a.tp = pv + to; a.tx = x + to; a.tr = r + to; a.tb = c->v_b.p + to; a.tD2 = tD2; a.tz = z + to; a.tS = c->v_S.p + to;
    a.step_partials = step;
    return a;
}

static int pcg_solve_fused(i3d_context* c, const i3d_optimizer_config& cfg, const OptParams& p, const PcgState** final_state) {
    hipStream_t s = c->stream;
    const Layout L = layout_of(c);
    const size_t to = L.tail_off; const Seg2 own = L.own;
    RowView r = c->row_view(); TilePlan tp = c->tile_plan();
    const bool sh = sharded(c);
    ShardArgs sa; std::memset(&sa, 0, sizeof(sa));
    if (sh) {
        if (!c->comm->fused_exchange(&sa.pd) || L.NS + 2 > sa.pd.L.red_cap) return ctx_fail(c, I3D_ERR_STATE, "pcg_solve_fused: the in-kernel exchanges are not available");
        const HaloPlan& h = c->halo;
        sa.rim = RimLists{h.n_send, h.n_recv, c->halo_send_idx.p, c->halo_send_peer.p, c->halo_recv_idx.p, c->halo_recv_peer.p, c->halo_offs.p, c->halo_offs.p + P2P_MAX_RANKS};
        sa.n_rim_wg = (h.n_send + h.n_recv) > 0 ? std::max(1, std::min(4, (std::max(h.n_send, h.n_recv) + 1023) / 1024)) : 1;
        sa.zb = c->v_z.p; sa.pb = c->v_p.p; sa.ub = c->v_u.p; sa.cmb = c->v_cm.p; sa.chunk = c->chunk;
    }
    const int wg_cap = sh ? sa.pd.wg_cap : 0;
    PcgState* const st2 = c->d_pcg2.p;
    const int NSP = (L.NS + 3) & ~3;
    double* const step_part = c->d_partials.p; double* const pq_part = c->d_partials.p + 4 * 2048; double* const d2_part = pq_part + 2048;
    { TimedScope t(c, I3D_K_VECTOR); launch_fill(s, (int)L.NP, c->v_x.p, 0.0f); launch_pcg_init3(s, st2, cfg.pcg_fixed_iterations, 500, c->d_lm.p); }
    CTX_HIP(c, hipMemcpyAsync(c->v_r.p, c->v_b.p, sizeof(float) * L.NP, hipMemcpyDeviceToDevice, s));
    Step3Args a = step3_args(c, L, p, tp, c->v_x.p, c->v_r.p, c->v_p.p, c->v_z.p, c->v_qacc.p, tp.qh, step_part, pq_part, d2_part, c->cam_part.p, c->Minv_blocks.p, c->v_D2.p + to, wg_cap);
    a.sharded = sh ? 1 : 0; a.lad_sys = -1;
    int n_step = 0;
    { TimedScope t(c, I3D_K_VECTOR); a.cur = st2; n_step = launch_pcg_step3(s, 0 , a); }
    const bool mr1 = c->mr1_serial && !sh && tp.T == 512 && tp.hp_off != nullptr && r.slots == 5;
    auto op = [&](double* pq, const PcgState* cur) -> int {
        if (mr1) { const int sys0[3] = {0, 0, 0}; LadVec z; std::memset(&z, 0, sizeof(z));
                   return launch_eg_tile_mr(s, r, p, tp, 1, sys0, c->v_u.p, c->v_qacc.p, tp.qh, pq, c->cam_part.p, NSP, cur, z); }
        return launch_eg_tile(s, r, p, c->v_u.p, tp, nullptr, c->v_qacc.p, pq, cur, c->cam_part.p, NSP);
    };
    const int seq0 = c->pcg_seq;
    int it = 1;
    for (;; ++it) {
        PcgState* const prev = st2 + ((it + 1) & 1); PcgState* const cur = st2 + (it & 1);
        sa.seq = seq0 + it; sa.n_slice_partials = a.n_slice_wg; a.sh = sa;
        { TimedScope t(c, I3D_K_VECTOR);
          a.n_d2 = launch_pcg_dir3(s, it == 1, own, to, L.NS, c->v_z.p, c->v_p.p, c->v_S.p, c->v_u.p, c->v_D2.p, c->v_cm.p, c->d_lm.p, step_part, n_step, d2_part, prev, cur, c->d_flags, seq0 + it,
                                   sh ? &sa : nullptr); }
        if (sh) { c->comm->count_reduce(4); c->comm->count_halo(c->halo.n_send); c->comm->count_reduce((size_t)L.NS + 1); }
        { TimedScope t(c, I3D_K_EG_PASS); a.n_pq = op(pq_part, cur); a.n_cam = a.n_pq; }
        a.cur = cur;
        if (it % 10 != 0) { TimedScope t(c, I3D_K_VECTOR); n_step = launch_pcg_step3(s, 1, a); }
        else {
            { TimedScope t(c, I3D_K_VECTOR); launch_pcg_step3(s, 2, a);
              launch_mul2(s, own, c->v_S.p, c->v_x.p, c->v_u.p); launch_mul(s, L.NS, c->v_S.p + to, c->v_x.p + to, c->v_u.p + to); }
            if (sh) { TimedScope t(c, I3D_K_COMM); launch_rim_u(s, sa, cur); c->comm->count_halo(c->halo.n_send); }
            { TimedScope t(c, I3D_K_EG_PASS); a.n_cam = op(nullptr, cur); }
            { TimedScope t(c, I3D_K_VECTOR); n_step = launch_pcg_step3(s, 3, a); }
        }
        if (it >= 2) {
            const int want = seq0 + it - 1; bool done = false;
            { const int rc = wait_pass(c, c->h_flags + 2 * (want & 1), want, "pcg_solve: the device stopped publishing its state", &done); if (rc) return rc; }
            if (done) break;
        }
        if (it > 520) break;
// ... 28 lines not shown
    if (!ok) {
        (void)hipGetLastError();
        c->lad_vec.release(); c->lad_qh.release(); c->lad_cam.release(); c->lad_part.release();
        std::fprintf(stderr, "[i3d] the slabs of the damping ladder (%d systems x %.1f MB) do not fit the device: this outer iteration runs the serial trust-region loop\n", nsys,
                     (double)(6 * vec + qh + cam) * 4.0 / 1e6);
        return 1;
    }
    return I3D_OK;
}
enum { LV_X = 0, LV_R, LV_P, LV_Z, LV_U, LV_Q };
static float* lad_vecp(const i3d_context* c, int kind, int sys = 0) { return c->lad_vec.p + ((size_t)kind * c->ladder_max + sys) * c->lad.vec; }

static int pcg_solve_ladder(i3d_context* c, const i3d_optimizer_config& cfg, const OptParams& p, int B, const PcgState** finals, int* passes_out) {
    hipStream_t s = c->stream;
    const Layout L = layout_of(c);
    const int K = c->K; const size_t to = L.tail_off; const Seg2 own = L.own;
    RowView r = c->row_view(); TilePlan tp = c->tile_plan();
    LadVec lv = c->lad;
    float* const X0 = lad_vecp(c, LV_X); float* const R0 = lad_vecp(c, LV_R); float* const P0 = lad_vecp(c, LV_P); float* const Z0 = lad_vecp(c, LV_Z);
    float* const U0 = lad_vecp(c, LV_U); float* const Q0 = lad_vecp(c, LV_Q);
    PcgState* const st2 = c->lad_st.p;
    const int NSP = (L.NS + 3) & ~3;
    double* const step_part0 = c->lad_part.p; double* const pq_part0 = step_part0 + LAD_PART_STEP; double* const d2_part0 = pq_part0 + LAD_PART_PQ;
    const bool use_mr = c->sw.ladder_mr;
    const bool mr1 = c->sw.ladder_mr1;
    const int mr_cap = std::min(c->sw.ladder_group, eg_tile_mr_max_systems(K));
    const bool pair = c->sw.ladder_pair;
    const bool mr_ok = use_mr && mr_cap >= 1 && tp.T == 512 && tp.hp_off != nullptr && r.slots == 5;
    const bool sh = sharded(c);
    double* const red4 = sh ? c->lad_red.p : nullptr;
    const int rstride = (int)lad_redop_stride(L.NS);
    double* const redop = sh ? c->lad_red.p + (size_t)LADDER_MAX * 4 : nullptr;
    { TimedScope t(c, I3D_K_VECTOR);
      for (int j = 0; j < B; ++j) { CTX_HIP(c, hipMemsetAsync(X0 + (size_t)j * lv.vec, 0, sizeof(float) * L.NP, s));
                                    CTX_HIP(c, hipMemcpyAsync(R0 + (size_t)j * lv.vec, c->v_b.p, sizeof(float) * L.NP, hipMemcpyDeviceToDevice, s)); }
      launch_pcg_init_lad(s, st2, B, cfg.pcg_fixed_iterations, 500, c->d_lm.p); }
    Step3Args a = step3_args(c, L, p, tp, X0, R0, P0, Z0, Q0, c->lad_qh.p, step_part0, pq_part0, d2_part0, c->lad_cam.p, c->lad_mblk.p, c->lad_tail.p, 0);
    a.sharded = 0; a.lad_sys = 0; a.redop = redop; a.redop_stride = rstride;
    std::vector<int> live(B); for (int j = 0; j < B; ++j) live[j] = j;
    auto set_slots = [&]() { for (int q = 0; q < LADDER_MAX; ++q) lv.sysid[q] = live[q < (int)live.size() ? q : (int)live.size() - 1]; };
    auto rows_apply = [&](int parity, bool with_dot) -> int {
        int n = 0; const int nl = (int)live.size();
        if (sh) { TimedScope t(c, I3D_K_COMM);
                  if (c->comm->push_halo_multi(U0, lv.vec, live.data(), nl, c->halo, s)) return -1; }
        if (mr_ok && (nl > 1 || mr1 || sh)) {
            const int groups = (nl + mr_cap - 1) / mr_cap;
            int at = 0;
            if (groups == 2 && pair && !sh && nl - (nl + 1) / 2 >= 2) {
                const int na = (nl + 1) / 2;
                TimedScope t(c, na == 2 ? I3D_K_EG_MR2 : I3D_K_EG_MR3);
                n = launch_eg_tile_mr_pair(s, r, p, tp, na, nl - na, live.data(), U0, Q0, c->lad_qh.p, with_dot ? pq_part0 : nullptr, c->lad_cam.p, NSP, st2 + parity, lv);
                if (n > 0) { at = nl; ++c->lad_streams; ++c->lad_paired; }
            }
            for (int g = 0; g < groups && at < nl; ++g) {
                const int ng = (nl - at + (groups - g) - 1) / (groups - g);
                TimedScope t(c, ng == 1 ? I3D_K_EG_PASS : (ng == 2 ? I3D_K_EG_MR2 : I3D_K_EG_MR3));
                n = launch_eg_tile_mr(s, r, p, tp, ng, live.data() + at, U0, Q0, c->lad_qh.p, with_dot ? pq_part0 : nullptr, c->lad_cam.p, NSP, st2 + parity, lv);
                if (n <= 0) return -1;
                at += ng; ++c->lad_streams;
            }
        } else {
            for (int j : live) {
                TilePlan tj = tp; tj.qh = c->lad_qh.p + (size_t)j * lv.qh;
                TimedScope t(c, I3D_K_EG_PASS);
                n = launch_eg_tile(s, r, p, U0 + (size_t)j * lv.vec, tj, nullptr, Q0 + (size_t)j * lv.vec, with_dot ? pq_part0 + (size_t)j * lv.part : nullptr, st2 + 2 * j + parity,
                                   c->lad_cam.p + (size_t)j * lv.cam, NSP);
                ++c->lad_streams;
            }
        }
        c->lad_system_passes += nl; ++c->lad_pass_live[nl < 6 ? nl : 6];
        if (sh) {
// ... 41 lines not shown
            }
            live.swap(still);
            if (live.empty()) break;
        }
        if (it > 520) break;
    }
    if (passes_out) *passes_out = it;
    c->pcg_seq = seq0 + PCG_SEQ_STRIDE;
    for (int j : live) finals[j] = st2 + 2 * j + (it & 1);
    { const int lrc = ctx_launch_check(c); if (lrc) return lrc; }
    return I3D_OK;
}

static int wait_record(i3d_context* c, int idx, int seq, LmRecord& out) {
    LmRecord* const r = c->h_lmrec + idx;
    const double t0 = now_s();
    while (__atomic_load_n(&r->seq, __ATOMIC_ACQUIRE) != seq) {
        if (now_s() - t0 > 60.0) {
            CTX_HIP(c, sync_stream(c));
            if (__atomic_load_n(&r->seq, __ATOMIC_ACQUIRE) != seq) return ctx_fail(c, I3D_ERR_HIP, "lm_solve: the device stopped publishing the state of the trust-region loop");
        }
    }
    out = *r;
    return I3D_OK;
}

static int lm_solve(i3d_context* c, const i3d_optimizer_config& cfg, OptParams& p, i3d_iteration_stats* st, double initial_radius) {
    hipStream_t s = c->stream;
    const Layout L = layout_of(c);
    const int N = c->N, K = c->K, NP = (int)L.NP, NS = L.NS;
    GridView g = c->grid_view(); RowView r = c->row_view();
    if (cfg.lm_steps > LM_REC_SLOTS - 2) return ctx_fail(c, I3D_ERR_CAPACITY, "optimize: more than 62 LM steps per outer iteration");
    { TimedScope t(c, I3D_K_VECTOR); launch_freemask(s, r, p, c->v_mask.p); }
    CTX_HIP(c, hipMemcpyAsync(c->xc_sdf.p, c->x_sdf.p, sizeof(double) * (size_t)N, hipMemcpyDeviceToDevice, s));
    CTX_HIP(c, hipMemcpyAsync(c->xc_alb.p, c->x_alb.p, sizeof(double) * (size_t)N, hipMemcpyDeviceToDevice, s));
    const bool one_stream = one_stream_gradcol(c);
    auto after_colnorm = [&]() -> int {
        CTX_HIP(c, hipMemcpyAsync(c->d_cam_c.p, c->d_shared.p, sizeof(double) * (size_t)NS, hipMemcpyDeviceToDevice, s));
        CTX_HIP(c, hipMemcpyAsync(c->d_cam_H.p, c->d_blocks.p, sizeof(double) * ((size_t)21 * K + 25), hipMemcpyDeviceToDevice, s));
        { int rc2 = allgather(c, c->v_c.p); if (rc2) return rc2; }
        { TimedScope t(c, I3D_K_VECTOR); launch_scale_from_colnorm(s, NP, c->v_c.p, c->v_mask.p, c->v_S.p, c->v_cm.p); }
        return I3D_OK;
    };
    int rc = I3D_OK;
    if (one_stream) { rc = run_gradcol(c, p, after_colnorm); if (rc) return rc; }
    else {
        rc = run_pass(c, PASS_COLNORM, p, nullptr, c->v_c.p); if (rc) return rc;
        rc = after_colnorm(); if (rc) return rc;
        rc = run_pass(c, PASS_GRAD, p, nullptr, c->v_acc.p); if (rc) return rc;
    }
    { TimedScope t(c, I3D_K_VECTOR); launch_mul(s, NP, c->v_S.p, c->v_acc.p, c->v_b.p); }
    if (!c->sw.cost0) { rc = eval_cost_launch(c, p, false, c->d_frames.p); if (rc) return rc; }
    else if (!one_stream) { TimedScope t(c, I3D_K_VECTOR); launch_set_double(s, c->d_scal.p + 16, c->cost_at_build); }
    rc = count_above_dev(c, c->v_acc.p, c->v_mask.p, 1e-10f, c->d_scal.p + 8); if (rc) return rc;
    rc = dot_dev(c, c->v_mask.p, c->v_mask.p, c->d_scal.p + 9); if (rc) return rc;
    {
        double* xs = c->h_pinned;
        for (int i = 0; i < 6 * K; ++i) xs[i] = c->poses[i];
        for (int i = 0; i < 4; ++i) xs[6 * K + i] = c->intr[i];
        for (int i = 0; i < 5; ++i) xs[6 * K + 4 + i] = c->dist[i];
        CTX_HIP(c, hipMemcpyAsync(c->d_xshared.p, xs, sizeof(double) * NS, hipMemcpyHostToDevice, s));
    }
    const int seq0 = c->lm_seq; c->lm_seq += LM_REC_SLOTS;
    LmState* const lm = c->d_lm.p;
    launch_lm_init(s, lm, c->d_scal.p + 16, c->d_scal.p + 8, c->d_scal.p + 9, initial_radius, c->d_lmrec, seq0);

    bool fused = c->tile_ok;
    if (fused && sharded(c)) { P2PDev probe; fused = c->comm->fused_exchange(&probe) && L.NS + 2 <= probe.L.red_cap; }
    int attempts = 0; bool ended = false, accepted = false;
    auto consume = [&](const LmRecord& rec) {
        if (rec.kind == 0) {
            if (st) { st->cost_initial = rec.cost; st->cost_final = rec.cost; st->free_parameters = (int64_t)(rec.nfree + 0.5); st->termination = rec.final_ ? 1 : 0; st->final_radius = initial_radius; }
            c->last_sizes[5] = (long long)(rec.nfree + 0.5);
        } else if (rec.kind == 2) { if (st) st->termination = 1; }
        else {
            if (st) {
                st->lm_iterations = attempts + 1;
                if (attempts < 50) { st->pcg_iterations[attempts] = rec.pcg_it; st->step_accepted[attempts] = rec.accepted; }
                st->final_radius = rec.radius_after; st->termination = rec.termination;
                if (rec.accepted) { st->cost_final = rec.cost; st->successful_steps += 1; }
            }
            if (cfg.verbose) std::printf("  [i3d LM] it %d cand %.9e model %.3e rho %.4f radius -> %.3e cg %d%s\n", attempts + 1, rec.cand_cost, rec.model_change, rec.rel, rec.radius_after, rec.pcg_it,
                                         rec.accepted ? " accepted" : "");
            accepted = rec.accepted != 0;
            ++attempts;
        }
        if (rec.final_) ended = true;
    };
    auto queue_decision = [&](const float* x, const PcgState* ps, int attempt, int lad_next) -> int {
        { TimedScope t(c, I3D_K_VECTOR);
          launch_candidate(s, g, r, K, -1.0f, x, c->v_S.p, c->d_xshared.p, c->xc_sdf.p, c->xc_alb.p, c->d_xcshared.p, c->d_scal.p + 4, c->v_mask.p, c->d_partials.p, lm);
          launch_cand_frames(s, K, c->d_xcshared.p, c->d_frames.p, c->d_frames_cand.p, lm); }
        const int rc2 = eval_cost_launch(c, p, true, c->d_frames_cand.p, c->d_xcshared.p + 6 * K, lm); if (rc2) return rc2;
        { TimedScope t(c, I3D_K_VECTOR);
          launch_lm_decide(s, lm, ps, c->d_scal.p + 4, c->d_scal.p + 16, attempt, cfg.lm_steps, c->d_lmrec + 1 + attempt, seq0 + 1 + attempt, lad_next,
                           c->sw.debug_invalid_attempt == attempt ? 1 : 0);
          launch_accept(s, g, r, c->xc_sdf.p, c->xc_alb.p, lm); }
        return I3D_OK;
    };
    bool ladder = c->ladder_max > 1 && c->tile_ok && (sharded(c) ? !fused : fused) && c->plan_T() == 512 && c->tile_plan().hp_off != nullptr && c->slots == 5;
    if (ladder && alloc_ladder(c) != I3D_OK) {
        ladder = false;
    }
    if (ladder) {
        const LadVec& lv = c->lad;
        { LmRecord rec; rc = wait_record(c, 0, seq0, rec); if (rc) return rc; consume(rec); }
        const bool warm = c->ladder_hint > 0;
        int k = 0, prevB = 0; bool after_resync = false;
        while (k < cfg.lm_steps && !ended) {
            int B = after_resync ? 1 : (prevB == 0 ? (warm ? std::max(c->ladder_hint, c->ladder_hint_prev) : 2) : (warm ? 2 : 2 * prevB));
            B = std::max(1, std::min(B, std::min(c->ladder_max, cfg.lm_steps - k)));
            after_resync = false; prevB = B;
            { TimedScope t(c, I3D_K_VECTOR);
              launch_lm_begin_lad(s, lm, B, K, p.fix_poses, p.fix_intr, p.fix_dist, c->d_cam_c.p, c->d_cam_H.p, c->lad_mblk.p, lv.mblk, c->v_c.p + L.tail_off, c->v_S.p + L.tail_off, c->lad_tail.p, lv.tail,
                                  c->d_lmrec + 1 + k, seq0 + 1 + k); }
            const PcgState* fin[LADDER_MAX] = {nullptr};
            rc = pcg_solve_ladder(c, cfg, p, B, fin, nullptr); if (rc) return rc;
            ++c->lad_batches;
            for (int j = 0; j < B && sharded(c); ++j) { rc = allgather(c, lad_vecp(c, LV_X, j)); if (rc) return rc; }
            for (int j = 0; j < B; ++j) { rc = queue_decision(lad_vecp(c, LV_X, j), fin[j], k + j, j + 1); if (rc) return rc; }
            int decided = 0;
            for (int j = 0; j < B && !ended; ++j) {
                LmRecord rec; rc = wait_record(c, 1 + k + j, seq0 + 1 + k + j, rec); if (rc) return rc;
                if (rec.kind == 3) {
                    __atomic_store_n(&c->h_lmrec[1 + k + j].seq, 0, __ATOMIC_RELEASE);
                    ++c->lad_resyncs; after_resync = true; break;
                }
                consume(rec); ++decided;
            }
            if (ended && decided < B) c->lad_wasted += B - decided;
            k += decided;
        }
        if (attempts > 0) { c->ladder_hint_prev = c->ladder_hint; c->ladder_hint = attempts; }
        ended = true;
    }
    int k = 0;
    for (; !ladder && k < cfg.lm_steps; ++k) {
        { TimedScope t(c, I3D_K_VECTOR);
          launch_lm_begin(s, lm, K, p.fix_poses, p.fix_intr, p.fix_dist, c->d_cam_c.p, c->d_cam_H.p, c->Minv_blocks.p, c->v_c.p + L.tail_off, c->v_S.p + L.tail_off, c->v_D2.p + L.tail_off, c->v_Minv.p + L.tail_off,
                          c->d_lmrec + 1 + k, seq0 + 1 + k);
          if (!fused) launch_lm_diag_dev(s, (int)L.tail_off, c->v_c.p, c->v_S.p, lm, c->v_D2.p, c->v_Minv.p); }
        const PcgState* ps = nullptr;
        rc = fused ? pcg_solve_fused(c, cfg, p, &ps) : pcg_solve(c, cfg, p, &ps); if (rc) return rc;
        { LmRecord rec; rc = wait_record(c, k, seq0 + k, rec); if (rc) return rc; consume(rec); }
        if (ended) break;
        { int rc2 = allgather(c, c->v_x.p); if (rc2) return rc2; }
        rc = queue_decision(c->v_x.p, ps, k, -1); if (rc) return rc;
    }
    if (!ended) { LmRecord rec; rc = wait_record(c, k, seq0 + k, rec); if (rc) return rc; consume(rec); }
    if (st) st->num_attempts = std::min(attempts, 50);
    CTX_HIP(c, hipMemcpyAsync(c->h_pinned, c->d_xcshared.p, sizeof(double) * NS, hipMemcpyDeviceToHost, s));
    CTX_HIP(c, sync_stream(c));
    if (sharded(c) && c->comm->health(s)) return ctx_fail(c, I3D_ERR_COMM, "lm_solve: a peer-to-peer exchange timed out (a rank stopped taking part)");
    if (accepted) {
        for (int i = 0; i < 6 * K; ++i) c->poses[i] = c->h_pinned[i];
        for (int i = 0; i < 4; ++i) c->intr[i] = c->h_pinned[6 * K + i];
        for (int i = 0; i < 5; ++i) c->dist[i] = c->h_pinned[6 * K + 4 + i];
    }
    { const int lrc = ctx_launch_check(c); if (lrc) return lrc; }
    return I3D_OK;
}

int optimize(i3d_context* c, const i3d_optimizer_config& cfg, i3d_iteration_stats* stats) {
    if (!c->have_grid || cfg.iterations < 1) return ctx_fail(c, I3D_ERR_INVALID_ARGUMENT, "optimize: no grid or iterations < 1");
    CTX_HIP(c, hipSetDevice(c->device));
    double carried_radius = 1e4;
    for (int itr = 0; itr < cfg.iterations; ++itr) {
        i3d_iteration_stats local; std::memset(&local, 0, sizeof(local));
        i3d_iteration_stats* st = stats ? &stats[itr] : &local;
        std::memset(st, 0, sizeof(*st));
        OptParams p;
        const double t0 = now_s();
        int rc = assemble(c, cfg, itr, p, st); if (rc) return rc;
        const double t1 = now_s();
        st->time_add = (c->t_add_end >= 0.0 && c->t_add_end <= t1 - t0) ? c->t_add_end : t1 - t0; st->time_build = (t1 - t0) - st->time_add;
        if (c->n_active > 0) { rc = lm_solve(c, cfg, p, st, cfg.carry_trust_radius ? carried_radius : 1e4); if (rc) return rc;
                               if (st->final_radius > 0.0) carried_radius = st->final_radius; }
        const double t2 = now_s();
        st->time_solve = t2 - t1;
        if (cfg.verbose) std::printf("[i3d] itr %d rows %lld/%lld/%lld/%lld valid %lld cost %.9e -> %.9e (add %.3f ms, solve %.3f ms)\n", itr,
                                     (long long)st->rows[0], (long long)st->rows[1], (long long)st->rows[2], (long long)st->rows[3], (long long)st->valid_voxels,
                                     st->cost_initial, st->cost_final, st->time_add * 1e3, st->time_solve * 1e3);
        timing_flush(c);
// ... 73 lines not shown
```

Before: 44.00.

## Fold small reductions into consumers and drop redundant copies and memsets

Several small launches and copies are removed. The candidate-norm and cost partial reductions are folded into a 1024-thread lm_decide kernel. PCG init writes x=0 and r=b itself instead of using a separate fill and memcpy. The full-grid xc mirror copy is replaced by a restore kernel that only touches active voxels when a step is rejected. Camera-matrix copies are skipped on the one-stream gradcol path, and dot/count reductions assign instead of memset-plus-accumulate. Together these cut launch count and device memcpy traffic per LM step, at the cost of more state (mirror_ok) that must stay consistent across calls.

```diff
diff --git a/intrinsic3d_amd/csrc/device/build.hip b/intrinsic3d_amd/csrc/device/build.hip
--- a/intrinsic3d_amd/csrc/device/build.hip
+++ b/intrinsic3d_amd/csrc/device/build.hip
@@ -505,8 +505,9 @@
 }
 
 void launch_build(hipStream_t st, GridView g, RowView r, OptParams p, const FrameConst* frames, bool with_jacobian, double* cost_out, double* scratch,
-                  const double* cam9, const LmState* lm) {
-    if (r.nC <= 0) { if (!with_jacobian && cost_out) (void)hipMemsetAsync(cost_out, 0, sizeof(double), st); return; }
+                  const double* cam9, const LmState* lm, int* n_partials) {
+    if (n_partials) *n_partials = 0;
+    if (r.nC <= 0) { if (!with_jacobian && cost_out && !n_partials) (void)hipMemsetAsync(cost_out, 0, sizeof(double), st); return; }
 #ifdef I3D_COST_MULTI_PROBE
     const int blocks = with_jacobian ? (r.nC + 255) / 256 : (((r.nC + 255) / 256 + 7) / 8) * 8 * I3D_COST_MULTI_PROBE;
 #else
@@ -528,7 +529,8 @@
         if (lds <= 48 * 1024) k_build<false, true, 2><<<blocks, 256, lds, st>>>(g, r, p, frames, cost_out, cam9, lm);
         else k_build<false, false, 2><<<blocks, 256, 0, st>>>(g, r, p, frames, cost_out, cam9, lm);
     }
-    if (!with_jacobian) launch_reduce_partials(st, scratch, blocks, 1, cost_dst, nullptr, true);
+    if (!with_jacobian && n_partials) *n_partials = blocks;
+    else if (!with_jacobian) launch_reduce_partials(st, scratch, blocks, 1, cost_dst, nullptr, true);
 }
 
 template <bool COST>
diff --git a/intrinsic3d_amd/csrc/device/gradcol.hip b/intrinsic3d_amd/csrc/device/gradcol.hip
--- a/intrinsic3d_amd/csrc/device/gradcol.hip
+++ b/intrinsic3d_amd/csrc/device/gradcol.hip
@@ -177,7 +177,7 @@
     if (!set_dynamic_lds((const void*)k_eg_gradcol, "k_eg_gradcol", n, p.K)) return 0;
     const int used = (ntiles + tiles_per_block - 1) / tiles_per_block;
     k_eg_gradcol<<<used, GC_THREADS, n, st>>>(g, r, p, b, tiles_per_block);
-    launch_reduce_partials(st, b.cost_partials, used, 1, b.cost_out, nullptr);
+    launch_reduce_partials(st, b.cost_partials, used, 1, b.cost_out, nullptr, true);
     return used;
 }
 
diff --git a/intrinsic3d_amd/csrc/device/kernels.hpp b/intrinsic3d_amd/csrc/device/kernels.hpp
--- a/intrinsic3d_amd/csrc/device/kernels.hpp
+++ b/intrinsic3d_amd/csrc/device/kernels.hpp
@@ -30,7 +30,7 @@
 void launch_group_cull(hipStream_t st, GridView g, RowView r, OptParams p, const FrameConst* frames, const float2* dblocks, float4* bounds, unsigned* mask);
 
 void launch_build(hipStream_t st, GridView g, RowView r, OptParams p, const FrameConst* frames, bool with_jacobian, double* cost_out , double* scratch,
-                  const double* cam9 = nullptr, const LmState* lm = nullptr);
+                  const double* cam9 = nullptr, const LmState* lm = nullptr, int* n_partials = nullptr);
 void launch_weight_sums(hipStream_t st, RowView r, GridView g, bool with_cost, double* sums13 , double* scratch);
 
 enum PassMode { PASS_GRAD = 0, PASS_JTJP = 1, PASS_COLNORM = 2 };
@@ -65,9 +65,9 @@
 void launch_mul(hipStream_t st, int n, const float* a, const float* b, float* out);
 void launch_scale_from_colnorm(hipStream_t st, int n, const float* c, const float* freemask, float* S, float* cm);
 void launch_dot(hipStream_t st, int n, const float* a, const float* b, double* out , double* scratch);
-void launch_count_above2(hipStream_t st, Seg2 sg, const float* a, const float* m, float tol, double* out, double* scratch);
+void launch_count_above2(hipStream_t st, Seg2 sg, const float* a, const float* m, float tol, double* out, double* scratch, bool assign = false);
 void launch_count_above(hipStream_t st, int n, const float* a, const float* m, float tol, double* out, double* scratch);
-void launch_dot2(hipStream_t st, Seg2 sg, const float* a, const float* b, double* out , double* scratch);
+void launch_dot2(hipStream_t st, Seg2 sg, const float* a, const float* b, double* out , double* scratch, bool assign = false);
 void launch_mul2(hipStream_t st, Seg2 sg, const float* a, const float* b, float* out);
 void launch_freemask(hipStream_t st, RowView r, OptParams p, float* mask );
 
@@ -104,6 +104,7 @@
 inline int tile_plan_hmax_of(int T) { return T == 1024 ? 2048 : 1536; }
 inline int tile_plan_tiles_of(int A, int T) { return (A + T - 1) / T; }
 size_t tile_plan_temp_bytes(size_t nslots);
+void launch_tile_plan_iota(hipStream_t st, size_t n, int* iota);
 hipError_t launch_tile_plan(hipStream_t st, RowView r, TilePlan t, int hmax_limit , void* temp, size_t temp_bytes);
 void launch_eaw_sym(hipStream_t st, RowView r, TilePlan t, const int* cflag );
 int  launch_eg_tile(hipStream_t st, RowView r, OptParams p, const float* u, TilePlan t, double* shared, float* qacc, double* pq_partials ,
@@ -147,6 +148,7 @@
     PcgState* cur;
     int sharded; ShardArgs sh;
     int lad_sys;
+    int init_xr;
     const double* redop; int redop_stride;
 };
 void launch_pcg_init3(hipStream_t st, PcgState* st2 , int fixed_iterations, int max_iterations, const LmState* lm = nullptr);
@@ -173,8 +175,10 @@
 size_t halo_sort_temp_bytes(int cap);
 hipError_t launch_halo_sort(hipStream_t st, void* temp, size_t temp_bytes, const unsigned long long* in, unsigned long long* out, int n);
 
-void launch_candidate(hipStream_t st, GridView g, RowView r, int K, float sign, const float* step, const float* S, const double* x_shared, double* xc_sdf, double* xc_alb,
-                      double* xc_shared, double* norms2 , const float* mask, double* scratch, const LmState* lm = nullptr);
+int  launch_candidate(hipStream_t st, GridView g, RowView r, int K, float sign, const float* step, const float* S, const double* x_shared, double* xc_sdf, double* xc_alb,
+                      double* xc_shared, double* norms2 , const float* mask, double* scratch, const LmState* lm = nullptr,
+                      bool reduce = true);
+void launch_mirror_restore(hipStream_t st, GridView g, RowView r, double* xc_sdf, double* xc_alb, const LmState* lm);
 void launch_accept(hipStream_t st, GridView g, RowView r, const double* xc_sdf, const double* xc_alb, const LmState* lm = nullptr);
 void launch_set_double(hipStream_t st, double* dst, double v);
 void launch_lm_init(hipStream_t st, LmState* lm, const double* cost, const double* ngrad, const double* nfree, double radius0, LmRecord* rec, int seq);
@@ -183,7 +187,8 @@
 void launch_lm_diag_dev(hipStream_t st, int n, const float* c, const float* S, const LmState* lm, float* D2, float* Minv);
 void launch_cand_frames(hipStream_t st, int K, const double* xc, const FrameConst* base, FrameConst* out, const LmState* lm);
 void launch_lm_decide(hipStream_t st, LmState* lm, const PcgState* ps, const double* norms2, const double* cand_cost, int attempt, int lm_steps, LmRecord* rec, int seq,
-                      int lad_next = -1 , int debug_invalid = 0);
+                      int lad_next = -1 , int debug_invalid = 0,
+                      const double* norm_partials = nullptr, int n_norm = 0, const double* cost_partials = nullptr, int n_cost = 0);
 void launch_lm_begin_lad(hipStream_t st, LmState* lm, int B, int K, int fix_poses, int fix_intr, int fix_dist, const double* cdiag, const double* tri, float* Mblk, size_t mblk_stride,
                          const float* tc, const float* tS, float* tD2, size_t tail_stride, LmRecord* rec, int seq);
 void launch_mark_compute(hipStream_t st, RowView r, int* flag);
diff --git a/intrinsic3d_amd/csrc/device/lm_kernels.hip b/intrinsic3d_amd/csrc/device/lm_kernels.hip
--- a/intrinsic3d_amd/csrc/device/lm_kernels.hip
+++ b/intrinsic3d_amd/csrc/device/lm_kernels.hip
@@ -1,5 +1,6 @@
 #include "kernels.hpp"
 #include "frame_math.hpp"
+#include "reduce_device.hpp"
 
 namespace i3d {
 
@@ -135,15 +136,24 @@
     if (K > 0) k_cand_frames<<<(K + 63) / 64, 64, 0, st>>>(K, xc, base, out, lm);
 }
 
-__global__ void k_lm_decide(LmState* lm, const PcgState* __restrict__ ps, const double* __restrict__ norms2, const double* __restrict__ cand_cost_p, int attempt , int lm_steps,
-                            LmRecord* rec, int seq, int lad_next, int debug_invalid) {
-    if (lm->done) return;
+__global__ void __launch_bounds__(1024) k_lm_decide(LmState* lm, const PcgState* __restrict__ ps, const double* __restrict__ norms2, const double* __restrict__ cand_cost_p, int attempt , int lm_steps,
+                                                    LmRecord* rec, int seq, int lad_next, int debug_invalid,
+                                                    const double* __restrict__ norm_partials, int n_norm, const double* __restrict__ cost_partials, int n_cost) {
+    __shared__ int done_s;
+    if (threadIdx.x == 0) done_s = lm->done;
+    __syncthreads();
+    if (done_s) return;
+    double nrm0 = 0.0, nrm1 = 0.0, cand = 0.0;
+    if (norm_partials) { nrm0 = reduce_partials_wg(norm_partials, n_norm, 2, 0); nrm1 = reduce_partials_wg(norm_partials, n_norm, 2, 1); }
+    if (cost_partials) cand = reduce_partials_wg(cost_partials, n_cost, 1, 0);
+    if (threadIdx.x != 0) return;
+    if (!norm_partials) { nrm0 = norms2[0]; nrm1 = norms2[1]; }
+    if (!cost_partials) cand = *cand_cost_p;
     const int pcg_it = ps->done == 2 ? ps->it + 1 : ps->it;
     const double xbr = ps->xbr, d2xx = ps->d2xx;
     const double model_change = 0.5 * xbr + 0.5 * d2xx;
     const bool finite = !(isnan(xbr) || isinf(xbr) || isnan(d2xx) || isinf(d2xx));
     double radius = lm->radius, decrease = lm->decrease_factor, cost = lm->cost;
-    const double cand = *cand_cost_p;
     int final_ = 0, accepted = 0, termination = lm->termination, invalid = lm->invalid, successful = lm->successful;
     double rel = 0.0;
     if (!finite || !(model_change > 0.0) || debug_invalid) {
@@ -151,7 +161,7 @@
         else radius *= 0.5;
     } else {
         invalid = 0;
-        const double step_norm = sqrt(norms2[0]), x_norm = sqrt(norms2[1]);
+        const double step_norm = sqrt(nrm0), x_norm = sqrt(nrm1);
         const double cost_change = cost - cand;
         if (step_norm <= 1e-8 * (x_norm + 1e-8)) { termination = 1; final_ = 1; }
         else if (fabs(cost_change) <= 1e-6 * cost) { termination = 1; final_ = 1; }
@@ -186,8 +196,9 @@
         }
     }
 }
-void launch_lm_decide(hipStream_t st, LmState* lm, const PcgState* ps, const double* norms2, const double* cand_cost, int attempt, int lm_steps, LmRecord* rec, int seq, int lad_next, int debug_invalid) {
-    k_lm_decide<<<1, 1, 0, st>>>(lm, ps, norms2, cand_cost, attempt, lm_steps, rec, seq, lad_next, debug_invalid);
-}
-
-}
+void launch_lm_decide(hipStream_t st, LmState* lm, const PcgState* ps, const double* norms2, const double* cand_cost, int attempt, int lm_steps, LmRecord* rec, int seq, int lad_next, int debug_invalid,
+                      const double* norm_partials, int n_norm, const double* cost_partials, int n_cost) {
+    k_lm_decide<<<1, (norm_partials || cost_partials) ? 1024 : 1, 0, st>>>(lm, ps, norms2, cand_cost, attempt, lm_steps, rec, seq, lad_next, debug_invalid, norm_partials, n_norm, cost_partials, n_cost);
+}
+
+}
diff --git a/intrinsic3d_amd/csrc/device/operator.hip b/intrinsic3d_amd/csrc/device/operator.hip
--- a/intrinsic3d_amd/csrc/device/operator.hip
+++ b/intrinsic3d_amd/csrc/device/operator.hip
@@ -10,15 +10,7 @@
 __global__ void __launch_bounds__(1024) k_reduce_partials(const double* __restrict__ partials, int nblk, int ncomp, double* dst, const PcgState* __restrict__ state, int assign) {
     if (state && state->done) return;
     for (int k = 0; k < ncomp; ++k) {
-        double s = 0.0;
-        for (int i0 = threadIdx.x; i0 < nblk; i0 += 8 * 1024) {
-            double v[8];
-#pragma unroll
-            for (int q = 0; q < 8; ++q) v[q] = partials[(size_t)min(i0 + q * 1024, nblk - 1) * ncomp + k];
-#pragma unroll
-            for (int q = 0; q < 8; ++q) if (i0 + q * 1024 < nblk) s += v[q];
-        }
-        const double t = block_sum_d(s);
+        const double t = reduce_partials_wg(partials, nblk, ncomp, k);
         if (threadIdx.x == 0) dst[k] = assign ? t : dst[k] + t;
     }
 }
@@ -511,17 +503,17 @@
     if (sg.n > 0) k_mul2<<<vblocks(2 * sg.n), 256, 0, st>>>(sg.n, sg.off1 - sg.off0, a + sg.off0, b + sg.off0, o + sg.off0);
 }
 void launch_scale_from_colnorm(hipStream_t st, int n, const float* c, const float* m, float* S, float* cm) { if (n > 0) k_scale<<<vblocks(n), 256, 0, st>>>(n, c, m, S, cm); }
-void launch_dot2(hipStream_t st, Seg2 sg, const float* a, const float* b, double* out, double* scratch) {
+void launch_dot2(hipStream_t st, Seg2 sg, const float* a, const float* b, double* out, double* scratch, bool assign) {
     if (sg.n <= 0) return;
     const int blocks = vblocks(2 * sg.n) > 1024 ? 1024 : vblocks(2 * sg.n);
     k_dot2<<<blocks, 256, 0, st>>>(sg.n, sg.off1 - sg.off0, a + sg.off0, b + sg.off0, scratch);
-    launch_reduce_partials(st, scratch, blocks, 1, out, nullptr);
-}
-void launch_count_above2(hipStream_t st, Seg2 sg, const float* a, const float* m, float tol, double* out, double* scratch) {
+    launch_reduce_partials(st, scratch, blocks, 1, out, nullptr, assign);
+}
+void launch_count_above2(hipStream_t st, Seg2 sg, const float* a, const float* m, float tol, double* out, double* scratch, bool assign) {
     if (sg.n <= 0) return;
     const int blocks = vblocks(2 * sg.n) > 1024 ? 1024 : vblocks(2 * sg.n);
     k_count_above2<<<blocks, 256, 0, st>>>(sg.n, sg.off1 - sg.off0, a + sg.off0, m + sg.off0, tol, scratch);
-    launch_reduce_partials(st, scratch, blocks, 1, out, nullptr);
+    launch_reduce_partials(st, scratch, blocks, 1, out, nullptr, assign);
 }
 void launch_count_above(hipStream_t st, int n, const float* a, const float* m, float tol, double* out, double* scratch) {
     if (n <= 0) return;
@@ -822,17 +814,23 @@
     }
     block_partial_d(d2, norms2, 2, 0); block_partial_d(x2, norms2, 2, 1);
 }
-void launch_candidate(hipStream_t st, GridView g, RowView r, int K, float sign, const float* step, const float* S, const double* xsh, double* xc_sdf, double* xc_alb,
-                      double* xc_sh, double* norms2, const float* mask, double* scratch, const LmState* lm) {
+int launch_candidate(hipStream_t st, GridView g, RowView r, int K, float sign, const float* step, const float* S, const double* xsh, double* xc_sdf, double* xc_alb,
+                     double* xc_sh, double* norms2, const float* mask, double* scratch, const LmState* lm, bool reduce) {
     int b = vblocks(r.A + 6 * K + 9); if (b > 1024) b = 1024;
     k_candidate<<<b, 256, 0, st>>>(g, r, K, sign, step, S, xsh, xc_sdf, xc_alb, xc_sh, scratch, mask, lm);
-    launch_reduce_partials(st, scratch, b, 2, norms2, nullptr, true);
+    if (reduce) launch_reduce_partials(st, scratch, b, 2, norms2, nullptr, true);
+    return b;
 }
 __global__ void k_accept(GridView g, RowView r, const double* __restrict__ xc_sdf, const double* __restrict__ xc_alb, const LmState* __restrict__ lm) {
     if (lm && !lm->accepted) return;
     GRID_STRIDE(r.A) { const int s = r.alist[i]; const double a = xc_sdf[s], b = xc_alb[s]; g.x_sdf[s] = a; g.x_alb[s] = b; g.f_sdf[s] = (float)a; g.f_alb[s] = (float)b; }
 }
 void launch_accept(hipStream_t st, GridView g, RowView r, const double* xc_sdf, const double* xc_alb, const LmState* lm) { if (r.A > 0) k_accept<<<vblocks(r.A), 256, 0, st>>>(g, r, xc_sdf, xc_alb, lm); }
+__global__ void k_mirror_restore(GridView g, RowView r, double* __restrict__ xc_sdf, double* __restrict__ xc_alb, const LmState* __restrict__ lm) {
+    if (lm->accepted) return;
+    GRID_STRIDE(r.A) { const int s = r.alist[i]; xc_sdf[s] = g.x_sdf[s]; xc_alb[s] = g.x_alb[s]; }
+}
+void launch_mirror_restore(hipStream_t st, GridView g, RowView r, double* xc_sdf, double* xc_alb, const LmState* lm) { if (r.A > 0) k_mirror_restore<<<vblocks(r.A), 256, 0, st>>>(g, r, xc_sdf, xc_alb, lm); }
 
 __global__ void k_halo_pack(int n, const int* __restrict__ idx, const float* __restrict__ vec, int chunk, float* __restrict__ buf) {
     const int i = blockIdx.x * blockDim.x + threadIdx.x;
diff --git a/intrinsic3d_amd/csrc/device/pcg_fused.hip b/intrinsic3d_amd/csrc/device/pcg_fused.hip
--- a/intrinsic3d_amd/csrc/device/pcg_fused.hip
+++ b/intrinsic3d_amd/csrc/device/pcg_fused.hip
@@ -238,7 +238,7 @@
     for (int seg = 0; seg < 2; ++seg) {
         const int i = q + seg * a.chunk4;
         v.cm[seg] = a.cm[i];
-        if (MODE == S3_INIT) v.r[seg] = r[i];
+        if (MODE == S3_INIT) v.r[seg] = a.init_xr ? a.b[i] : r[i];
         else {
             v.x[seg] = x[i];
             if (MODE != S3_RESET) v.p[seg] = p[i];
@@ -265,7 +265,21 @@
     __shared__ int done_s;
     if (threadIdx.x == 0) done_s = cur->done;
     __syncthreads();
-    if (done_s) return;
+    if (done_s) {
+        if (MODE == S3_INIT && a.init_xr) {
+            if (slice_wg) {
+                for (int q = q0; q < a.nq; q += qstride) {
+#pragma unroll
+                    for (int seg = 0; seg < 2; ++seg) { const int i = q + seg * a.chunk4; X[i] = make_float4(0.0f, 0.0f, 0.0f, 0.0f); R[i] = a.b[i]; }
+                }
+            } else {
+                const int K = a.K, tw = (int)blockIdx.x - a.n_slice_wg, n_pose_wg = (K + PF_POSES_PER_WG - 1) / PF_POSES_PER_WG;
+                const int col0 = tw < n_pose_wg ? 6 * PF_POSES_PER_WG * tw : 6 * K, ncol = tw < n_pose_wg ? min(6 * K, col0 + 6 * PF_POSES_PER_WG) - col0 : 9;
+                if ((int)threadIdx.x < ncol) { const int i = col0 + threadIdx.x; tr[i] = a.tb[i]; tx[i] = 0.0f; }
+            }
+        }
+        return;
+    }
     const float inv_radius = o.sys >= 0 ? a.lm->lad_inv_radius[o.sys] : a.lm->inv_radius;
     float alpha = 0.0f;
     if (MODE == S3_NORMAL || MODE == S3_XONLY) {
@@ -316,7 +330,8 @@
                 float xv[4], rv[4], svv[4], dv[4], mv[4];
                 { const float4 cv = in.cm[seg]; lm_from_colnorm(cv.x, inv_radius, svv[0], dv[0], mv[0]); lm_from_colnorm(cv.y, inv_radius, svv[1], dv[1], mv[1]);
                   lm_from_colnorm(cv.z, inv_radius, svv[2], dv[2], mv[2]); lm_from_colnorm(cv.w, inv_radius, svv[3], dv[3], mv[3]); }
-                if (MODE == S3_INIT) { const float4 t = in.r[seg]; rv[0] = t.x; rv[1] = t.y; rv[2] = t.z; rv[3] = t.w; }
+                if (MODE == S3_INIT) { const float4 t = in.r[seg]; rv[0] = t.x; rv[1] = t.y; rv[2] = t.z; rv[3] = t.w;
+                                       if (a.init_xr) { X[i] = make_float4(0.0f, 0.0f, 0.0f, 0.0f); R[i] = t; } }
                 else {
                     const float4 xo = in.x[seg];
                     xv[0] = xo.x; xv[1] = xo.y; xv[2] = xo.z; xv[3] = xo.w;
@@ -373,7 +388,7 @@
             const int i = col0 + t;
             const bool fixed = i < 6 * K ? a.fix_poses : (i < 6 * K + 4 ? a.fix_intr : a.fix_dist);
             float ri;
-            if (MODE == S3_INIT) ri = tr[i];
+            if (MODE == S3_INIT) { if (a.init_xr) { ri = a.tb[i]; tr[i] = ri; tx[i] = 0.0f; } else ri = tr[i]; }
             else {
                 float xi = tx[i];
                 if (MODE != S3_RESET) { xi += alpha * tp[i]; tx[i] = xi; }
diff --git a/intrinsic3d_amd/csrc/device/reduce_device.hpp b/intrinsic3d_amd/csrc/device/reduce_device.hpp
--- a/intrinsic3d_amd/csrc/device/reduce_device.hpp
+++ b/intrinsic3d_amd/csrc/device/reduce_device.hpp
@@ -18,4 +18,16 @@
     if (threadIdx.x == 0) partials[(size_t)blockIdx.x * ncomp + comp] = t;
 }
 
+static __device__ inline double reduce_partials_wg(const double* __restrict__ partials, int nblk, int ncomp, int k) {
+    double s = 0.0;
+    for (int i0 = threadIdx.x; i0 < nblk; i0 += 8 * 1024) {
+        double v[8];
+#pragma unroll
+        for (int q = 0; q < 8; ++q) v[q] = partials[(size_t)min(i0 + q * 1024, nblk - 1) * ncomp + k];
+#pragma unroll
+        for (int q = 0; q < 8; ++q) if (i0 + q * 1024 < nblk) s += v[q];
+    }
+    return block_sum_d(s);
 }
+
+}
diff --git a/intrinsic3d_amd/csrc/device/tile_pass.hip b/intrinsic3d_amd/csrc/device/tile_pass.hip
--- a/intrinsic3d_amd/csrc/device/tile_pass.hip
+++ b/intrinsic3d_amd/csrc/device/tile_pass.hip
@@ -506,6 +506,7 @@
 }
 
 __global__ void k_iota(int n, int* __restrict__ x) { const int i = blockIdx.x * blockDim.x + threadIdx.x; if (i < n) x[i] = i; }
+void launch_tile_plan_iota(hipStream_t st, size_t n, int* iota) { if (n > 0) k_iota<<<(unsigned)((n + 255) / 256), 256, 0, st>>>((int)n, iota); }
 
 size_t tile_plan_temp_bytes(size_t nslots) {
     size_t bytes = 0;
@@ -531,7 +532,6 @@
         else { if (t.ntiles_own > 0) k_tile_pull_plan<512, 1536><<<t.ntiles_own, 512, 0, st>>>(r, t.tile_first, nullptr, t.lnbr, t.halo_cnt, off, src, t.overflow);
                if (t.n_ghost > 0) k_tile_pull_plan<512, 1536><<<t.n_ghost, 512, 0, st>>>(r, 0, t.ghost_tiles, t.lnbr, t.halo_cnt, off, src, t.overflow); }
     }
-    k_iota<<<(n + 255) / 256, 256, 0, st>>>(n, t.iota);
     int key_bits = 32;
     for (int b = 1; b < 32; ++b) { const unsigned mask = (1u << b) - 1u; if ((1u << b) >= (unsigned)r.A && ((unsigned)TP_NONE & mask) >= (unsigned)r.A) { key_bits = b; break; } }
     e = rocprim::radix_sort_pairs(temp, temp_bytes, (const int*)t.halo_idx, t.ext_e, (const int*)t.iota, t.ext_pos, (size_t)n, 0, key_bits, st);
diff --git a/intrinsic3d_amd/csrc/host/context.cpp b/intrinsic3d_amd/csrc/host/context.cpp
--- a/intrinsic3d_amd/csrc/host/context.cpp
+++ b/intrinsic3d_amd/csrc/host/context.cpp
@@ -144,6 +144,7 @@
 
 namespace i3d {
 int set_grid_device(i3d_context* c, int N, float voxel_size, float truncation, GridStaging& g) {
+    c->mirror_ok = false;
     c->N = N; c->voxel_size = voxel_size; c->truncation = truncation; c->have_grid = false; c->have_sh = false; c->have_subvolumes = false; c->assembled = false;
     c->render_bricks_ok = false;
     c->slots = 0;
@@ -165,6 +166,7 @@
                         c->x_sdf.p, c->x_alb.p, c->f_sdf.p, c->f_alb.p, c->weight.p, c->color.p);
     CTX_HIP(c, hipMemcpyAsync(c->xc_sdf.p, c->x_sdf.p, sizeof(double) * (size_t)N, hipMemcpyDeviceToDevice, st));
     CTX_HIP(c, hipMemcpyAsync(c->xc_alb.p, c->x_alb.p, sizeof(double) * (size_t)N, hipMemcpyDeviceToDevice, st));
+    c->mirror_ok = true;
     unsigned int cap = 1; while (cap < (unsigned int)N * 2u) cap <<= 1;
     CTX_HIP(c, fit(c->hkeys, cap)); CTX_HIP(c, fit(c->hvals, cap)); c->hmask = cap - 1;
     CTX_HIP(c, hipMemsetAsync(c->hkeys.p, 0xff, sizeof(unsigned long long) * (size_t)cap, st));
@@ -204,6 +206,7 @@
     if (sdf_refined) { CTX_HIP(c, a.alloc(N)); CTX_HIP(c, hipMemcpyAsync(a.p, sdf_refined, sizeof(double) * (size_t)N, hipMemcpyHostToDevice, c->stream)); }
     if (albedo) { CTX_HIP(c, b.alloc(N)); CTX_HIP(c, hipMemcpyAsync(b.p, albedo, sizeof(double) * (size_t)N, hipMemcpyHostToDevice, c->stream)); }
     if (color) { CTX_HIP(c, col.alloc((size_t)3 * N)); CTX_HIP(c, hipMemcpyAsync(col.p, color, (size_t)3 * N, hipMemcpyHostToDevice, c->stream)); }
+    c->mirror_ok = false;
     launch_update_fields(c->stream, N, c->rank.p, a.p, b.p, col.p, c->x_sdf.p, c->x_alb.p, c->f_sdf.p, c->f_alb.p, c->color.p);
     CTX_HIP(c, hipStreamSynchronize(c->stream));
     c->assembled = false;
diff --git a/intrinsic3d_amd/csrc/host/context.hpp b/intrinsic3d_amd/csrc/host/context.hpp
--- a/intrinsic3d_amd/csrc/host/context.hpp
+++ b/intrinsic3d_amd/csrc/host/context.hpp
@@ -160,6 +160,7 @@
     int N = 0; float voxel_size = 0, truncation = 0;
     i3d::DevBuf<int> cx, cy, cz, rank, nbr, aidx, alist, aflag, ascan;
     i3d::DevBuf<double> sdf0, x_sdf, x_alb, xc_sdf, xc_alb;
+    bool mirror_ok = false;
     i3d::DevBuf<float> f_sdf, f_alb, weight, sh;
     i3d::DevBuf<uchar4> color;
     i3d::DevBuf<uint8_t> flags;
@@ -234,6 +235,7 @@
     int* h_flags = nullptr; int* d_flags = nullptr; int pcg_seq = 1024;
     i3d::DevBuf<i3d::LmState> d_lm; i3d::LmRecord* h_lmrec = nullptr; i3d::LmRecord* d_lmrec = nullptr; int lm_seq = 1;
     i3d::DevBuf<double> d_cam_c, d_cam_H;
+    i3d::DevBuf<double> d_cand_part;
     hipEvent_t ev_asm[2] = {nullptr, nullptr};
     long long n_syncs = 0;
     double* h_pinned = nullptr; size_t h_pinned_n = 0;
diff --git a/intrinsic3d_amd/csrc/host/solver.cpp b/intrinsic3d_amd/csrc/host/solver.cpp
--- a/intrinsic3d_amd/csrc/host/solver.cpp
+++ b/intrinsic3d_amd/csrc/host/solver.cpp
@@ -62,6 +62,7 @@
       const size_t nt = (size_t)tile_plan_tiles_of((int)Acap, 512);
       const size_t nh = std::max(nt * (size_t)tile_plan_hmax_of(512), (size_t)tile_plan_tiles_of((int)Acap, 1024) * (size_t)tile_plan_hmax_of(1024));
       CTX_HIP(c, c->tp_lnbr.alloc(Acap * LNBR_WORDS)); CTX_HIP(c, c->tp_eaw.alloc(Acap * 6)); CTX_HIP(c, c->tp_halo_idx.alloc(nh)); CTX_HIP(c, c->tp_halo_cnt.alloc(nt)); CTX_HIP(c, c->tp_iota.alloc(nh));
+      launch_tile_plan_iota(c->stream, c->tp_iota.n, c->tp_iota.p);
       CTX_HIP(c, c->tp_ext_e.alloc(nh)); CTX_HIP(c, c->tp_ext_pos.alloc(nh)); CTX_HIP(c, c->tp_qh.alloc(2 * nh)); CTX_HIP(c, c->tp_overflow.alloc(1));
       CTX_HIP(c, c->tp_ext_off.alloc(Acap + (size_t)SHARD_ALIGN * ((c->comm ? c->comm->world : 1) + 1) + 8));
       CTX_HIP(c, c->cam_part.alloc((size_t)2048 * (((size_t)6 * c->K + 9 + 3) & ~(size_t)3)));
@@ -88,7 +89,7 @@
     if (!c->h_flags) { CTX_HIP(c, hipHostMalloc((void**)&c->h_flags, 32 * sizeof(int), hipHostMallocMapped | hipHostMallocCoherent));
                        for (int i = 0; i < 32; ++i) c->h_flags[i] = -1;
                        CTX_HIP(c, hipHostGetDevicePointer((void**)&c->d_flags, c->h_flags, 0)); }
-    CTX_HIP(c, c->d_lm.alloc(1)); CTX_HIP(c, c->d_cam_c.alloc((size_t)6 * c->K + 9)); CTX_HIP(c, c->d_cam_H.alloc((size_t)21 * c->K + 25));
+    CTX_HIP(c, c->d_lm.alloc(1)); CTX_HIP(c, c->d_cam_c.alloc((size_t)6 * c->K + 9)); CTX_HIP(c, c->d_cam_H.alloc((size_t)21 * c->K + 25)); CTX_HIP(c, c->d_cand_part.alloc(2 * 1024));
     if (!c->h_lmrec) { CTX_HIP(c, hipHostMalloc((void**)&c->h_lmrec, LM_REC_SLOTS * sizeof(LmRecord), hipHostMallocMapped | hipHostMallocCoherent));
                        std::memset(c->h_lmrec, 0, LM_REC_SLOTS * sizeof(LmRecord));
                        CTX_HIP(c, hipHostGetDevicePointer((void**)&c->d_lmrec, c->h_lmrec, 0)); }
@@ -362,22 +363,24 @@
     return I3D_OK;
 }
 
-template <class F> static int run_gradcol(i3d_context* c, const OptParams& p, F between) {
+template <class F> static int run_gradcol(i3d_context* c, const OptParams& p, double* col_shared, double* col_blocks, F between) {
     hipStream_t s = c->stream; GridView g = c->grid_view(); RowView r = c->row_view(); const Layout L = layout_of(c);
     const int stride = (int)gc_part_stride(c->K), col_off = (int)gc_col_off(c->K);
     GradColBuffers gb{c->C.p, c->C2.p, c->treg.p, c->treg2.p, c->gc_part.p, stride, col_off, c->d_partials.p, c->d_scal.p + 16};
-    CTX_HIP(c, hipMemsetAsync(c->d_scal.p + 16, 0, sizeof(double), s));
-    CTX_HIP(c, hipMemsetAsync(c->d_shared.p, 0, sizeof(double) * ((size_t)L.NS + 1), s));
-    CTX_HIP(c, hipMemsetAsync(c->d_blocks.p, 0, sizeof(double) * (21 * (size_t)c->K + 25), s));
     int rows = 0;
     { TimedScope t(c, I3D_K_EG_AUX); rows = launch_eg_gradcol(s, g, r, p, gb);
       if (rows > GC_PART_ROWS) return ctx_fail(c, I3D_ERR_CAPACITY, "run_gradcol: more workgroups than rows of the camera partial buffer");
-      if (rows > 0) launch_sum_rows(s, PASS_COLNORM, c->K, c->gc_part.p + col_off, rows, stride, c->d_shared.p, c->d_blocks.p); }
-    { PassBuffers b{c->C2.p, c->treg2.p, c->d_shared.p, c->d_blocks.p, nullptr, 0};
+      if (rows > 0) launch_sum_rows(s, PASS_COLNORM, c->K, c->gc_part.p + col_off, rows, stride, col_shared, col_blocks); }
+    if (rows <= 0) {
+        CTX_HIP(c, hipMemsetAsync(c->d_scal.p + 16, 0, sizeof(double), s));
+        CTX_HIP(c, hipMemsetAsync(col_shared, 0, sizeof(double) * (size_t)L.NS, s));
+        CTX_HIP(c, hipMemsetAsync(col_blocks, 0, sizeof(double) * (21 * (size_t)c->K + 25), s));
+    }
+    { PassBuffers b{c->C2.p, c->treg2.p, col_shared, col_blocks, nullptr, 0};
       TimedScope t(c, I3D_K_GATHER); launch_gather(s, PASS_COLNORM, r, b, c->v_c.p); }
-    { TimedScope t(c, I3D_K_VECTOR); launch_shared_finalize(s, L.tail_off, c->K, p, c->d_shared.p, c->v_c.p, false, nullptr, nullptr, nullptr, nullptr, nullptr); }
+    { TimedScope t(c, I3D_K_VECTOR); launch_shared_finalize(s, L.tail_off, c->K, p, col_shared, c->v_c.p, false, nullptr, nullptr, nullptr, nullptr, nullptr); }
     { int rc = between(); if (rc) return rc; }
-    CTX_HIP(c, hipMemsetAsync(c->d_shared.p, 0, sizeof(double) * ((size_t)L.NS + 1), s));
+    if (rows <= 0) CTX_HIP(c, hipMemsetAsync(c->d_shared.p, 0, sizeof(double) * ((size_t)L.NS + 1), s));
     { TimedScope t(c, I3D_K_EG_AUX); if (rows > 0) launch_sum_rows(s, PASS_GRAD, c->K, c->gc_part.p, rows, stride, c->d_shared.p, c->d_blocks.p); }
     { PassBuffers b{c->C.p, c->treg.p, c->d_shared.p, c->d_blocks.p, nullptr, 0};
       TimedScope t(c, I3D_K_GATHER); launch_gather(s, PASS_GRAD, r, b, c->v_acc.p); }
@@ -387,8 +390,9 @@
 
 static int dot_dev(i3d_context* c, const float* a, const float* b, double* slot) {
     const Layout L = layout_of(c);
-    CTX_HIP(c, hipMemsetAsync(slot, 0, sizeof(double), c->stream));
-    { TimedScope t(c, I3D_K_VECTOR); launch_dot2(c->stream, L.own, a, b, slot, c->d_partials.p); }
+    const bool assign = L.own.n > 0;
+    if (!assign) CTX_HIP(c, hipMemsetAsync(slot, 0, sizeof(double), c->stream));
+    { TimedScope t(c, I3D_K_VECTOR); launch_dot2(c->stream, L.own, a, b, slot, c->d_partials.p, assign); }
     { int rc = allreduce(c, slot, 1); if (rc) return rc; }
     { TimedScope t(c, I3D_K_VECTOR); launch_dot(c->stream, L.NS, a + L.tail_off, b + L.tail_off, slot, c->d_partials.p); }
     return I3D_OK;
@@ -396,18 +400,19 @@
 
 static int count_above_dev(i3d_context* c, const float* a, const float* m, float tol, double* slot) {
     const Layout L = layout_of(c);
-    CTX_HIP(c, hipMemsetAsync(slot, 0, sizeof(double), c->stream));
-    { TimedScope t(c, I3D_K_VECTOR); launch_count_above2(c->stream, L.own, a, m, tol, slot, c->d_partials.p); }
+    const bool assign = L.own.n > 0;
+    if (!assign) CTX_HIP(c, hipMemsetAsync(slot, 0, sizeof(double), c->stream));
+    { TimedScope t(c, I3D_K_VECTOR); launch_count_above2(c->stream, L.own, a, m, tol, slot, c->d_partials.p, assign); }
     { int rc = allreduce(c, slot, 1); if (rc) return rc; }
     { TimedScope t(c, I3D_K_VECTOR); launch_count_above(c->stream, L.NS, a + L.tail_off, m + L.tail_off, tol, slot, c->d_partials.p); }
     return I3D_OK;
 }
 
-static int eval_cost_launch(i3d_context* c, const OptParams& p, bool candidate, const FrameConst* frames, const double* cam9 = nullptr, const LmState* lm = nullptr) {
+static int eval_cost_launch(i3d_context* c, const OptParams& p, bool candidate, const FrameConst* frames, const double* cam9 = nullptr, const LmState* lm = nullptr, int* n_partials = nullptr) {
     GridView g = c->grid_view();
     if (candidate) { g.x_sdf = c->xc_sdf.p; g.x_alb = c->xc_alb.p; }
-    { TimedScope t(c, I3D_K_COST); launch_build(c->stream, g, c->row_view(), p, frames, false, c->d_scal.p + 16, c->d_partials.p, cam9, lm); }
-    return allreduce(c, c->d_scal.p + 16, 1);
+    { TimedScope t(c, I3D_K_COST); launch_build(c->stream, g, c->row_view(), p, frames, false, c->d_scal.p + 16, c->d_partials.p, cam9, lm, n_partials); }
+    return n_partials ? I3D_OK : allreduce(c, c->d_scal.p + 16, 1);
 }
 static int eval_cost(i3d_context* c, const OptParams& p, bool candidate, const FrameConst* frames, double* cost) {
     int rc = eval_cost_launch(c, p, candidate, frames); if (rc) return rc;
@@ -544,10 +549,10 @@
     PcgState* const st2 = c->d_pcg2.p;
     const int NSP = (L.NS + 3) & ~3;
     double* const step_part = c->d_partials.p; double* const pq_part = c->d_partials.p + 4 * 2048; double* const d2_part = pq_part + 2048;
-    { TimedScope t(c, I3D_K_VECTOR); launch_fill(s, (int)L.NP, c->v_x.p, 0.0f); launch_pcg_init3(s, st2, cfg.pcg_fixed_iterations, 500, c->d_lm.p); }
-    CTX_HIP(c, hipMemcpyAsync(c->v_r.p, c->v_b.p, sizeof(float) * L.NP, hipMemcpyDeviceToDevice, s));
+    { TimedScope t(c, I3D_K_VECTOR); if (sh) launch_fill(s, (int)L.NP, c->v_x.p, 0.0f); launch_pcg_init3(s, st2, cfg.pcg_fixed_iterations, 500, c->d_lm.p); }
+    if (sh) CTX_HIP(c, hipMemcpyAsync(c->v_r.p, c->v_b.p, sizeof(float) * L.NP, hipMemcpyDeviceToDevice, s));
     Step3Args a = step3_args(c, L, p, tp, c->v_x.p, c->v_r.p, c->v_p.p, c->v_z.p, c->v_qacc.p, tp.qh, step_part, pq_part, d2_part, c->cam_part.p, c->Minv_blocks.p, c->v_D2.p + to, wg_cap);
-    a.sharded = sh ? 1 : 0; a.lad_sys = -1;
+    a.sharded = sh ? 1 : 0; a.lad_sys = -1; a.init_xr = sh ? 0 : 1;
     int n_step = 0;
     { TimedScope t(c, I3D_K_VECTOR); a.cur = st2; n_step = launch_pcg_step3(s, 0 , a); }
     const bool mr1 = c->mr1_serial && !sh && tp.T == 512 && tp.hp_off != nullptr && r.slots == 5;
@@ -642,11 +647,11 @@
     const int rstride = (int)lad_redop_stride(L.NS);
     double* const redop = sh ? c->lad_red.p + (size_t)LADDER_MAX * 4 : nullptr;
     { TimedScope t(c, I3D_K_VECTOR);
-      for (int j = 0; j < B; ++j) { CTX_HIP(c, hipMemsetAsync(X0 + (size_t)j * lv.vec, 0, sizeof(float) * L.NP, s));
-                                    CTX_HIP(c, hipMemcpyAsync(R0 + (size_t)j * lv.vec, c->v_b.p, sizeof(float) * L.NP, hipMemcpyDeviceToDevice, s)); }
+      for (int j = 0; j < B && sh; ++j) { CTX_HIP(c, hipMemsetAsync(X0 + (size_t)j * lv.vec, 0, sizeof(float) * L.NP, s));
+                                          CTX_HIP(c, hipMemcpyAsync(R0 + (size_t)j * lv.vec, c->v_b.p, sizeof(float) * L.NP, hipMemcpyDeviceToDevice, s)); }
       launch_pcg_init_lad(s, st2, B, cfg.pcg_fixed_iterations, 500, c->d_lm.p); }
     Step3Args a = step3_args(c, L, p, tp, X0, R0, P0, Z0, Q0, c->lad_qh.p, step_part0, pq_part0, d2_part0, c->lad_cam.p, c->lad_mblk.p, c->lad_tail.p, 0);
-    a.sharded = 0; a.lad_sys = 0; a.redop = redop; a.redop_stride = rstride;
+    a.sharded = 0; a.lad_sys = 0; a.redop = redop; a.redop_stride = rstride; a.init_xr = sh ? 0 : 1;
     std::vector<int> live(B); for (int j = 0; j < B; ++j) live[j] = j;
     auto set_slots = [&]() { for (int q = 0; q < LADDER_MAX; ++q) lv.sysid[q] = live[q < (int)live.size() ? q : (int)live.size() - 1]; };
     auto rows_apply = [&](int parity, bool with_dot) -> int {
@@ -754,18 +759,23 @@
     GridView g = c->grid_view(); RowView r = c->row_view();
     if (cfg.lm_steps > LM_REC_SLOTS - 2) return ctx_fail(c, I3D_ERR_CAPACITY, "optimize: more than 62 LM steps per outer iteration");
     { TimedScope t(c, I3D_K_VECTOR); launch_freemask(s, r, p, c->v_mask.p); }
-    CTX_HIP(c, hipMemcpyAsync(c->xc_sdf.p, c->x_sdf.p, sizeof(double) * (size_t)N, hipMemcpyDeviceToDevice, s));
-    CTX_HIP(c, hipMemcpyAsync(c->xc_alb.p, c->x_alb.p, sizeof(double) * (size_t)N, hipMemcpyDeviceToDevice, s));
+    if (!c->mirror_ok) {
+        CTX_HIP(c, hipMemcpyAsync(c->xc_sdf.p, c->x_sdf.p, sizeof(double) * (size_t)N, hipMemcpyDeviceToDevice, s));
+        CTX_HIP(c, hipMemcpyAsync(c->xc_alb.p, c->x_alb.p, sizeof(double) * (size_t)N, hipMemcpyDeviceToDevice, s));
+    }
+    c->mirror_ok = false;
     const bool one_stream = one_stream_gradcol(c);
     auto after_colnorm = [&]() -> int {
-        CTX_HIP(c, hipMemcpyAsync(c->d_cam_c.p, c->d_shared.p, sizeof(double) * (size_t)NS, hipMemcpyDeviceToDevice, s));
-        CTX_HIP(c, hipMemcpyAsync(c->d_cam_H.p, c->d_blocks.p, sizeof(double) * ((size_t)21 * K + 25), hipMemcpyDeviceToDevice, s));
+        if (!one_stream) {
+            CTX_HIP(c, hipMemcpyAsync(c->d_cam_c.p, c->d_shared.p, sizeof(double) * (size_t)NS, hipMemcpyDeviceToDevice, s));
+            CTX_HIP(c, hipMemcpyAsync(c->d_cam_H.p, c->d_blocks.p, sizeof(double) * ((size_t)21 * K + 25), hipMemcpyDeviceToDevice, s));
+        }
         { int rc2 = allgather(c, c->v_c.p); if (rc2) return rc2; }
         { TimedScope t(c, I3D_K_VECTOR); launch_scale_from_colnorm(s, NP, c->v_c.p, c->v_mask.p, c->v_S.p, c->v_cm.p); }
         return I3D_OK;
     };
     int rc = I3D_OK;
-    if (one_stream) { rc = run_gradcol(c, p, after_colnorm); if (rc) return rc; }
+    if (one_stream) { rc = run_gradcol(c, p, c->d_cam_c.p, c->d_cam_H.p, after_colnorm); if (rc) return rc; }
     else {
         rc = run_pass(c, PASS_COLNORM, p, nullptr, c->v_c.p); if (rc) return rc;
         rc = after_colnorm(); if (rc) return rc;
@@ -810,13 +820,17 @@
         if (rec.final_) ended = true;
     };
     auto queue_decision = [&](const float* x, const PcgState* ps, int attempt, int lad_next) -> int {
+        const bool fold = !sharded(c);
+        int n_norm = 0, n_cost = 0;
         { TimedScope t(c, I3D_K_VECTOR);
-          launch_candidate(s, g, r, K, -1.0f, x, c->v_S.p, c->d_xshared.p, c->xc_sdf.p, c->xc_alb.p, c->d_xcshared.p, c->d_scal.p + 4, c->v_mask.p, c->d_partials.p, lm);
+          n_norm = launch_candidate(s, g, r, K, -1.0f, x, c->v_S.p, c->d_xshared.p, c->xc_sdf.p, c->xc_alb.p, c->d_xcshared.p, c->d_scal.p + 4, c->v_mask.p,
+                                    fold ? c->d_cand_part.p : c->d_partials.p, lm, !fold);
           launch_cand_frames(s, K, c->d_xcshared.p, c->d_frames.p, c->d_frames_cand.p, lm); }
-        const int rc2 = eval_cost_launch(c, p, true, c->d_frames_cand.p, c->d_xcshared.p + 6 * K, lm); if (rc2) return rc2;
+        const int rc2 = eval_cost_launch(c, p, true, c->d_frames_cand.p, c->d_xcshared.p + 6 * K, lm, fold ? &n_cost : nullptr); if (rc2) return rc2;
         { TimedScope t(c, I3D_K_VECTOR);
           launch_lm_decide(s, lm, ps, c->d_scal.p + 4, c->d_scal.p + 16, attempt, cfg.lm_steps, c->d_lmrec + 1 + attempt, seq0 + 1 + attempt, lad_next,
-                           c->sw.debug_invalid_attempt == attempt ? 1 : 0);
+                           c->sw.debug_invalid_attempt == attempt ? 1 : 0,
+                           fold ? c->d_cand_part.p : nullptr, n_norm, fold ? c->d_partials.p : nullptr, n_cost);
           launch_accept(s, g, r, c->xc_sdf.p, c->xc_alb.p, lm); }
         return I3D_OK;
     };
@@ -871,6 +885,8 @@
     }
     if (!ended) { LmRecord rec; rc = wait_record(c, k, seq0 + k, rec); if (rc) return rc; consume(rec); }
     if (st) st->num_attempts = std::min(attempts, 50);
+    { TimedScope t(c, I3D_K_VECTOR); launch_mirror_restore(s, g, r, c->xc_sdf.p, c->xc_alb.p, lm); }
+    c->mirror_ok = true;
     CTX_HIP(c, hipMemcpyAsync(c->h_pinned, c->d_xcshared.p, sizeof(double) * NS, hipMemcpyDeviceToHost, s));
     CTX_HIP(c, sync_stream(c));
     if (sharded(c) && c->comm->health(s)) return ctx_fail(c, I3D_ERR_COMM, "lm_solve: a peer-to-peer exchange timed out (a rank stopped taking part)");
```

Result: no change. 44.26, median of 6 (+0.6%).
